# loicland/superpoint_graph

Measured on AMD Instinct MI355X. Metric: superpoints/sec (embed+ECC fwd+bwd), S3DIS-shaped SPG, higher is better.
Workload: dtype f32; 1 GPU; gru_10_0,f_13 fwd+bwd+Adam; 1 scene/GPU x 1000 sp x 128 pts x 14 f, 5000 edges x 13 f; hipgraph=False, step_call=spg_train_step (one library call: forward + backward), parallelism=single GPU, batchnorm=per-rank statistics, precision=f32

## Files before the change

### include/spg_hip.h

```cpp
#ifndef SPG_HIP_H
#define SPG_HIP_H
#include <stddef.h>
#include <stdint.h>

#ifdef __cplusplus
extern "C" {
#endif

#define SPG_MAX_LAYERS 8
#define SPG_VERSION 200

const char* spg_last_error(void);
int spg_version(void);

size_t spg_graph_workspace_bytes(int N, int n_src, int E);
int spg_graph_build(const int64_t* idxn, const int64_t* degs, int N, int n_src, int E, void* graph_ws, void* stream);
int spg_graph_export(const void* graph_ws, int N, int n_src, int E, int32_t* rowptr, int32_t* src, int32_t* dst,
                     int32_t* rev_rowptr, int32_t* rev_eid, int32_t* hdr, void* stream);

int spg_ecc_aggregate_fwd(int dtype, const void* x, const void* w, const int64_t* idxe, const void* graph_ws, int N,
                          int E, int cin, int cout, int w_is_matrix, void* out, void* stream);
int spg_ecc_aggregate_bwd(int dtype, const void* x, const void* w, const int64_t* idxe, const void* graph_ws, int N,
                          int E, int n_x_rows, int n_w_rows, int cin, int cout, int w_is_matrix, const void* grad_out,
                          void* grad_x, void* grad_w, void* stream);
// ... 47 lines not shown
                             const float* ext_transform, const void* const* params, float* emb, void* workspace, int training,
                             int bn_update_times, void* stream);
int spg_pointnet_backward_ext(const spg_pointnet_cfg* cfg, int B, const float* clouds, const float* clouds_global,
                              const float* ext_transform, const void* const* params, const float* grad_emb, void* const* grads,
                              float* grad_transform, float* grad_global, void* workspace, void* bwd_workspace, void* stream);

#define SPG_MAX_PARTS 64
typedef struct spg_eccrnn_cfg {
  int nc, nrepeats, matrix, layernorm, ingate, cat_all;
  int n_fnet;
  int fnet_widths[SPG_MAX_LAYERS + 1];
  int bnidx, llbias;
  float bn_eps, bn_momentum;
  int cell;
  int n_parts;
  int part_ptr[SPG_MAX_PARTS + 1];
} spg_eccrnn_cfg;

size_t spg_eccrnn_workspace_bytes(const spg_eccrnn_cfg* cfg, int N, int E, int training);
int spg_eccrnn_forward(const spg_eccrnn_cfg* cfg, int N, int E, const void* graph_ws, const float* h0,
                       const float* edgefeats, const void* const* params, float* out, void* workspace, int training,
                       int bn_update_times, void* stream);
long spg_eccrnn_debug_offset(const spg_eccrnn_cfg* cfg, int N, int E, int training, int layer, int what);
size_t spg_eccrnn_bwd_workspace_bytes(const spg_eccrnn_cfg* cfg, int N, int E);
int spg_eccrnn_backward(const spg_eccrnn_cfg* cfg, int N, int E, const void* graph_ws, const float* edgefeats,
                        const void* const* params, const float* grad_out, float* grad_h0, void* const* grads,
                        void* workspace, void* bwd_workspace, void* stream);

#define SPG_LOADER_MAX_FEATS 16
int spg_load_superpoints(const float* points, int ncols, const int64_t* offsets, int n_superpoints, const int32_t* slot,
                         const int32_t* sample_idx, int npts, int xyznormalize, const int32_t* colmap, int nfeat,
                         const double* M, const float* noise, float* clouds, float* diam, void* stream);

size_t spg_set_batch_workspace_bytes(int N, int E);
int spg_set_batch(const int64_t* edges, int N, int E, int64_t* idxn, int64_t* degs, int64_t* perm, void* workspace,
                  int32_t* error_flag, void* stream);
int spg_gather_rows(const float* src, long ld_src, const int64_t* perm, long rows, int cols, float* dst, long ld_dst,
                    void* stream);

enum { SPG_EF_COPY = 0, SPG_EF_DIFF = 1, SPG_EF_LOGDIFF = 2, SPG_EF_RATIO = 3, SPG_EF_CONST = 4 };
#define SPG_EF_MAX_COLS 32
typedef struct {
  const void* data;
  long ld;
  int column, kind, is_f64, pad_;
} spg_edge_feature_spec;
typedef struct {
  int ncols, pad_;
  spg_edge_feature_spec col[SPG_EF_MAX_COLS];
} spg_edge_feature_specs;
int spg_edge_features(const spg_edge_feature_specs* specs, const int64_t* edges, long E, const double* mean,
                      const double* scale, float* out, void* stream);

size_t spg_batch_graph_scratch_bytes(int N, int E, int F);
int spg_batch_graph_build(const int64_t* edges_host, const float* feats_host, int N, int E, int F, int64_t* idxn, int64_t* degs,
                          float* feats_sorted, void* graph_ws, void* scratch, int32_t* error_flag, void* stream);
int spg_batch_graph_build_dev(const int64_t* edges_dev, const float* feats_dev, int N, int E, int F, int64_t* idxn, int64_t* degs,
                              float* feats_sorted, void* graph_ws, void* scratch, int32_t* error_flag, void* stream);
int spg_upload_packed(const void* const* host, const size_t* bytes, const size_t* offsets, int n, void* device, size_t total, void* stream);

int spg_upload(const void* host, size_t bytes, void* device, void* stream);

size_t spg_spg_workspace_bytes(int which, long n);
int spg_spg_tet_edges(const int32_t* tets, long T, const int32_t* comp, uint64_t* keys, long capacity, uint64_t* count, void* stream);
int spg_spg_unique_edges(const uint64_t* keys, long n, const float* xyz, const int32_t* comp, long n_com, float d_max,
                         uint64_t* edge_keys, uint64_t* cc_keys, uint64_t* count, void* workspace, size_t workspace_bytes, void* stream);
int spg_spg_group_edges(const uint64_t* cc_keys, const uint64_t* edge_keys, long n, uint64_t* cc_sorted, uint64_t* edges_sorted,
                        uint64_t* seg_cc, int64_t* seg_off, int64_t* n_seg, void* workspace, size_t workspace_bytes, void* stream);
int spg_spg_superpoints(const float* xyz, long n, const int32_t* comp, int n_com, const int32_t* labels, const uint32_t* label_rows,
                        int n_labels, float* centroids, float* length, float* surface, float* volume, uint64_t* point_count,
                        uint32_t* sp_labels, void* workspace, size_t workspace_bytes, void* stream);
int spg_spg_superedges(const uint64_t* edges_sorted, const uint64_t* seg_cc, const int64_t* seg_off, long n_sedg, long n_com,
                       const float* xyz, const float* centroids, const float* length, const float* surface, const float* volume,
                       const uint64_t* point_count, uint32_t* source, uint32_t* target, float* delta_mean, float* delta_std,
                       float* delta_norm, float* delta_centroid, float* length_ratio, float* surface_ratio, float* volume_ratio,
                       float* point_count_ratio, void* stream);
int spg_compute_geof(const float* xyz, const uint32_t* target, long n, int k_nn, float* geof, void* stream);

size_t spg_prune_workspace_bytes(long n);
int spg_prune_voxels(const float* xyz, long n, float voxel_size, int64_t* n_voxels, int32_t* error_flag, void* workspace,
                     size_t workspace_bytes, void* stream);
int spg_prune_reduce(const float* xyz, const uint8_t* rgb, const uint8_t* labels, const uint32_t* objects, long n, long n_voxels,
                     int n_labels, int n_objects, float* out_xyz, uint8_t* out_rgb, uint32_t* out_labels, uint32_t* out_objects,
                     int32_t* error_flag, void* workspace, size_t workspace_bytes, void* stream);

size_t spg_knn_workspace_bytes(long n_ref, long n_query, int k);
int spg_knn_build(const float* ref_xyz, long n_ref, float cell_size, int32_t* error_flag, void* workspace, size_t workspace_bytes,
                  void* stream);
int spg_knn_query(const float* query_xyz, long n_query, long n_ref, int k, int self_query, int32_t* idx_out, float* dist_out,
                  int32_t* error_flag, void* workspace, size_t workspace_bytes, void* stream);
long spg_knn_query_chunk(long n_ref, long n_query, size_t workspace_bytes);

size_t spg_edgegraph_workspace_bytes(long n, long E);
int spg_edgegraph_build(const int64_t* src, const int64_t* tgt, long E, long n, int32_t* rowptr, uint32_t* inc, int32_t* ends,
                        int32_t* error_flag, void* workspace, size_t workspace_bytes, void* stream);
size_t spg_edge_forward_workspace_bytes(long E);
int spg_edge_forward(int mode, const float* emb, long n, int d, const int32_t* ends, long E, int dist_type, int intra, int inter,
                     const uint8_t* is_transition, const float* weights, float* diff, float* dx, float* dl, double* loss_out,
                     void* workspace, size_t workspace_bytes, void* stream);
int spg_edge_loss_backward(const float* dl, const uint8_t* is_transition, const float* up, long E, float* grad_diff, void* stream);
int spg_edge_backward(const float* emb, long n, int d, const int32_t* rowptr, const uint32_t* inc, const int32_t* ends, long E,
                      int dist_type, const float* dl, const uint8_t* is_transition, const float* up, const float* grad_diff,
                      const float* dx, float* grad_emb, void* stream);
size_t spg_cc_workspace_bytes(long n);
int spg_connected_components(const int32_t* ends, const uint8_t* active, long E, long n, int32_t* in_component,
                             int32_t* component_size, int32_t* n_components, void* workspace, size_t workspace_bytes, void* stream);
size_t spg_xpart_workspace_bytes(long n, long E);
int spg_xpart_weights(const int32_t* ends, long E, long n, const int32_t* pred_in_component, const uint8_t* is_transition,
                      double factor, float* weights, int32_t* in_component, int32_t* component_size, int32_t* n_components,
                      void* workspace, size_t workspace_bytes, void* stream);

int spg_loader_random(const int64_t* counts, const int64_t* ids, const int32_t* slot, int n_superpoints, int npts, int nfeat,
                      uint64_t seed, uint32_t step, int augment, float scale, int rot, float mirror_prob, int jitter,
                      int32_t* sample_idx, double* M, float* noise, void* stream);

int spg_cross_entropy_fwd(const float* logits, const int64_t* target, const float* weight, int N, int C, int64_t ignore_index,
                          int reduction_mean, float* loss, float* lse, float* wsum, void* stream);
int spg_cross_entropy_bwd(const float* logits, const int64_t* target, const float* weight, const float* lse, const float* wsum,
                          const float* grad_loss, int N, int C, int64_t ignore_index, int reduction_mean, float* grad_logits,
                          void* stream);

int spg_eval_accumulate(const float* logits, int n_samples, long sample_stride, int N, int C, const int64_t* label_mode,
                        const int64_t* label_vec, int64_t* pred, int64_t* confusion, int64_t* counters, void* stream);

typedef int (*spg_allreduce_fn)(void* ctx, double* buf, long n, void* stream);
int spg_set_bn_allreduce(spg_allreduce_fn fn, void* ctx, double* buf, long buf_doubles);
typedef int (*spg_slot_allreduce_fn)(void* ctx, unsigned long long* words, long nwords, void* stream);
int spg_set_slot_allreduce(spg_slot_allreduce_fn fn, void* ctx, int world);

int spg_rccl_unique_id(void* out_128_bytes);
int spg_rccl_init(const void* unique_id_128_bytes, int world_size, int rank);
int spg_rccl_world_size(void);
int spg_rccl_allreduce_sum_f32(float* buf, long n, void* stream);
int spg_rccl_sync_bn(double* buf, long buf_doubles);
int spg_rccl_sync_slots(int on);
int spg_rccl_allreduce_sum_f64(double* buf, long n, void* stream);
int spg_rccl_destroy(void);

int spg_adam_clamp_step(float* param, float* grad, float* exp_avg, float* exp_avg_sq, long n, float lr, float beta1,
                        float beta2, float eps, float weight_decay, float grad_clip, int step, void* stream);
int spg_adam_clamp_step_scaled(float* param, float* grad, float* exp_avg, float* exp_avg_sq, long n, float lr, float beta1,
                               float beta2, float eps, float weight_decay, float grad_clip, int step, const float* grad_div,
                               void* stream);
int spg_adam_clamp_step_guarded(float* param, float* grad, float* exp_avg, float* exp_avg_sq, long n, float lr, float beta1,
                                float beta2, float eps, float weight_decay, float grad_clip, int step, const float* grad_div,
                                const float* guard_all, void* stream);
int spg_ecc_persistent_flag(float* dst, void* stream);

void spg_prof_enable(int on);
int spg_prof_read(double* ms, long* launches, double* flops, int reset);
int spg_prof_tag(int kind, int it, int jt, int x, int y, int full);
int spg_prof_read_shapes(int* keys, double* vals, int max);
int spg_tune(int key, int value);
typedef struct spg_step_args {
  const spg_pointnet_cfg* ptn_cfg;
  int B, bn_update_times;
  const float* clouds;
  const float* clouds_global;
  const void* const* ptn_params;
  void* const* ptn_grads;
  void* ptn_ws; void* ptn_bwd_ws;
  float* emb;
  float* grad_emb;
  int N, nf;
  const int64_t* slot_of_row;
  const int64_t* idx_valid;
  float* desc;
  float* grad_desc;
  const spg_eccrnn_cfg* ecc_cfg;
  int E;
  const void* graph_ws;
  const float* edgefeats;
  const void* const* ecc_params;
  void* const* ecc_grads;
  void* ecc_ws; void* ecc_bwd_ws;
  float* ecc_out;
  float* grad_ecc_out;
  int nout, n_classes;
  const float* cls_W; const float* cls_b;
  float* cls_dW; float* cls_db;
  float* cls_work;
  float* logits;
  float* grad_logits;
  const int64_t* target;
  const float* class_weight;
  int64_t ignore_index;
  int reduction_mean;
  float* loss_buf;
  int ptn_slots_clean;
} spg_step_args;
int spg_train_step(const spg_step_args* args, void* stream);
int spg_infer_step(const spg_step_args* args, void* stream);
int spg_cross_entropy_fwd_bwd(const float* logits, const int64_t* target, const float* weight, int N, int C, int64_t ignore_index,
                              int reduction_mean, float* loss, float* lse, float* wsum, float* grad_logits, void* stream);

int spg_ecc_persistent_errors(void);
int spg_ecc_persistent_errors_clear(void);
int spg_ecc_persistent_status(int* errors, int* withheld, int clear);
int spg_prof_read_tag(int tag, double* ms, long* launches, double* flops);

int spg_group_trace(void* buf, int max_launches);
int spg_group_trace_read(int* out, int max);

#ifdef __cplusplus
}
#endif
#endif
```

### superpoint_graph_amd/_lib.py

```python
from __future__ import annotations

import ctypes
import os
import subprocess

import torch

_HERE = os.path.dirname(os.path.abspath(__file__))
CSRC = os.path.join(_HERE, 'csrc')
LIB_PATH = os.environ.get('SPG_HIP_LIB') or os.path.join(CSRC, 'libspg_hip.so')

SPG_MAX_LAYERS = 8
SPG_MAX_PARTS = 64
c_void_pp = ctypes.POINTER(ctypes.c_void_p)


class PointNetCfg(ctypes.Structure):
    _fields_ = [('nfeat', ctypes.c_int), ('nfeat_stn', ctypes.c_int), ('nfeat_global', ctypes.c_int), ('npts', ctypes.c_int),
                ('n_stn_conv', ctypes.c_int), ('n_stn_fc', ctypes.c_int), ('n_conv', ctypes.c_int), ('n_fc', ctypes.c_int),
                ('stn_conv', ctypes.c_int * SPG_MAX_LAYERS), ('stn_fc', ctypes.c_int * SPG_MAX_LAYERS),
                ('conv', ctypes.c_int * SPG_MAX_LAYERS), ('fc', ctypes.c_int * SPG_MAX_LAYERS),
                ('last_ac', ctypes.c_int), ('bn_eps', ctypes.c_float), ('bn_momentum', ctypes.c_float)]


class EccRnnCfg(ctypes.Structure):
    _fields_ = [('nc', ctypes.c_int), ('nrepeats', ctypes.c_int), ('matrix', ctypes.c_int), ('layernorm', ctypes.c_int),
                ('ingate', ctypes.c_int), ('cat_all', ctypes.c_int), ('n_fnet', ctypes.c_int),
                ('fnet_widths', ctypes.c_int * (SPG_MAX_LAYERS + 1)), ('bnidx', ctypes.c_int), ('llbias', ctypes.c_int),
                ('bn_eps', ctypes.c_float), ('bn_momentum', ctypes.c_float), ('cell', ctypes.c_int),
                ('n_parts', ctypes.c_int), ('part_ptr', ctypes.c_int * (SPG_MAX_PARTS + 1))]


_i, _l, _p, _sz = ctypes.c_int, ctypes.c_long, ctypes.c_void_p, ctypes.c_size_t

SPG_EF_MAX_COLS = 32


class EdgeFeatureSpec(ctypes.Structure):
    _fields_ = [('data', ctypes.c_void_p), ('ld', ctypes.c_long), ('column', ctypes.c_int), ('kind', ctypes.c_int),
                ('is_f64', ctypes.c_int), ('pad_', ctypes.c_int)]


class StepArgs(ctypes.Structure):
    _fields_ = [('ptn_cfg', ctypes.POINTER(PointNetCfg)), ('B', ctypes.c_int), ('bn_update_times', ctypes.c_int),
                ('clouds', ctypes.c_void_p), ('clouds_global', ctypes.c_void_p), ('ptn_params', c_void_pp), ('ptn_grads', c_void_pp),
                ('ptn_ws', ctypes.c_void_p), ('ptn_bwd_ws', ctypes.c_void_p), ('emb', ctypes.c_void_p), ('grad_emb', ctypes.c_void_p),
                ('N', ctypes.c_int), ('nf', ctypes.c_int), ('slot_of_row', ctypes.c_void_p), ('idx_valid', ctypes.c_void_p),
                ('desc', ctypes.c_void_p), ('grad_desc', ctypes.c_void_p),
                ('ecc_cfg', ctypes.POINTER(EccRnnCfg)), ('E', ctypes.c_int), ('graph_ws', ctypes.c_void_p), ('edgefeats', ctypes.c_void_p),
                ('ecc_params', c_void_pp), ('ecc_grads', c_void_pp), ('ecc_ws', ctypes.c_void_p), ('ecc_bwd_ws', ctypes.c_void_p),
                ('ecc_out', ctypes.c_void_p), ('grad_ecc_out', ctypes.c_void_p),
                ('nout', ctypes.c_int), ('n_classes', ctypes.c_int), ('cls_W', ctypes.c_void_p), ('cls_b', ctypes.c_void_p),
                ('cls_dW', ctypes.c_void_p), ('cls_db', ctypes.c_void_p), ('cls_work', ctypes.c_void_p), ('logits', ctypes.c_void_p),
                ('grad_logits', ctypes.c_void_p),
                ('target', ctypes.c_void_p), ('class_weight', ctypes.c_void_p), ('ignore_index', ctypes.c_int64),
                ('reduction_mean', ctypes.c_int), ('loss_buf', ctypes.c_void_p), ('ptn_slots_clean', ctypes.c_int)]


class EdgeFeatureSpecs(ctypes.Structure):
    _fields_ = [('ncols', ctypes.c_int), ('pad_', ctypes.c_int), ('col', EdgeFeatureSpec * SPG_EF_MAX_COLS)]


SIGNATURES = {
    'spg_last_error': (ctypes.c_char_p, []),
    'spg_version': (_i, []),
    'spg_graph_workspace_bytes': (_sz, [_i, _i, _i]),
    'spg_graph_build': (_i, [_p, _p, _i, _i, _i, _p, _p]),
    'spg_graph_export': (_i, [_p, _i, _i, _i, _p, _p, _p, _p, _p, _p, _p]),
    'spg_ecc_aggregate_fwd': (_i, [_i, _p, _p, _p, _p, _i, _i, _i, _i, _i, _p, _p]),
    'spg_ecc_aggregate_bwd': (_i, [_i, _p, _p, _p, _p, _i, _i, _i, _i, _i, _i, _i, _p, _p, _p, _p]),
    'spg_gru_scratch_floats': (_sz, [_i]),
    'spg_gru_cell_fwd': (_i, [_p, _p, _i, c_void_pp, _i, _i, _p, _p, _p]),
    'spg_gru_cell_bwd': (_i, [_p, _p, _p, _i, c_void_pp, _i, _i, _p, _p, c_void_pp, _p, _p]),
    'spg_lstm_scratch_floats': (_sz, [_i]),
    'spg_lstm_cell_fwd': (_i, [_p, _p, _p, _i, c_void_pp, _i, _i, _p, _p, _p, _p]),
    'spg_lstm_cell_bwd': (_i, [_p, _p, _p, _p, _p, _i, c_void_pp, _i, _i, _p, _p, _p, c_void_pp, _p, _p]),
    'spg_linear_fwd': (_i, [_p, _l, _i, _i, _p, _p, _i, _p, _p, _i, _p, _l, _p]),
    'spg_linear_dgrad': (_i, [_p, _l, _i, _i, _p, _i, _p, _l, _p]),
    'spg_colsum': (_i, [_p, _l, _l, _i, _p, _p, _p]),
    'spg_linear_wgrad_work_floats': (_sz, [_i, _i, _i]),
    'spg_linear_wgrad': (_i, [_p, _l, _p, _l, _i, _i, _i, _p, _p, _i, _p, _p, _p]),
    'spg_linear_wgrad_bias_work_floats': (ctypes.c_size_t, [_i, _i, _i]),
    'spg_linear_wgrad_bias': (_i, [_p, _l, _p, _l, _i, _i, _i, _p, _p, _i, _p, _p, _p, _p]),
    'spg_linear_backward': (_i, [_p, _l, _p, _l, _p, _i, _i, _i, _p, _l, _p, _p, _p, _p]),
    'spg_pointnet_num_layers': (_i, [ctypes.POINTER(PointNetCfg)]),
    'spg_pointnet_workspace_bytes': (_sz, [ctypes.POINTER(PointNetCfg), _i, _i]),
    'spg_pointnet_forward': (_i, [ctypes.POINTER(PointNetCfg), _i, _p, _p, c_void_pp, _p, _p, _i, _i, _p]),
    'spg_pointnet_forward_ext': (_i, [ctypes.POINTER(PointNetCfg), _i, _p, _p, _p, c_void_pp, _p, _p, _i, _i, _p]),
    'spg_pointnet_backward_ext': (_i, [ctypes.POINTER(PointNetCfg), _i, _p, _p, _p, c_void_pp, _p, c_void_pp, _p, _p, _p, _p, _p]),
    'spg_pointnet_debug_offset': (_l, [ctypes.POINTER(PointNetCfg), _i, _i, _i, _i]),
    'spg_pointnet_bwd_workspace_bytes': (_sz, [ctypes.POINTER(PointNetCfg), _i]),
    'spg_pointnet_backward': (_i, [ctypes.POINTER(PointNetCfg), _i, _p, _p, c_void_pp, _p, c_void_pp, _p, _p, _p]),
    'spg_eccrnn_workspace_bytes': (_sz, [ctypes.POINTER(EccRnnCfg), _i, _i, _i]),
    'spg_eccrnn_forward': (_i, [ctypes.POINTER(EccRnnCfg), _i, _i, _p, _p, _p, c_void_pp, _p, _p, _i, _i, _p]),
    'spg_eccrnn_bwd_workspace_bytes': (_sz, [ctypes.POINTER(EccRnnCfg), _i, _i]),
    'spg_eccrnn_debug_offset': (_l, [ctypes.POINTER(EccRnnCfg), _i, _i, _i, _i, _i]),
    'spg_ecc_persistent_errors': (_i, []),
    'spg_ecc_persistent_errors_clear': (_i, []),
    'spg_ecc_persistent_status': (_i, [ctypes.POINTER(ctypes.c_int), ctypes.POINTER(ctypes.c_int), _i]),
    'spg_eccrnn_backward': (_i, [ctypes.POINTER(EccRnnCfg), _i, _i, _p, _p, c_void_pp, _p, _p, c_void_pp, _p, _p, _p]),
    'spg_adam_clamp_step': (_i, [_p, _p, _p, _p, _l, ctypes.c_float, ctypes.c_float, ctypes.c_float, ctypes.c_float,
                                 ctypes.c_float, ctypes.c_float, _i, _p]),
    'spg_adam_clamp_step_scaled': (_i, [_p, _p, _p, _p, _l, ctypes.c_float, ctypes.c_float, ctypes.c_float, ctypes.c_float,
                                        ctypes.c_float, ctypes.c_float, _i, _p, _p]),
    'spg_adam_clamp_step_guarded': (_i, [_p, _p, _p, _p, _l, ctypes.c_float, ctypes.c_float, ctypes.c_float, ctypes.c_float,
                                        ctypes.c_float, ctypes.c_float, _i, _p, _p, _p]),
    'spg_ecc_persistent_flag': (_i, [_p, _p]),
    'spg_load_superpoints': (_i, [_p, _i, _p, _i, _p, _p, _i, _i, _p, _i, _p, _p, _p, _p, _p]),
    'spg_set_batch_workspace_bytes': (_sz, [_i, _i]),
    'spg_set_batch': (_i, [_p, _i, _i, _p, _p, _p, _p, _p, _p]),
    'spg_gather_rows': (_i, [_p, _l, _p, _l, _i, _p, _l, _p]),
    'spg_upload': (_i, [_p, _sz, _p, _p]),
    'spg_batch_graph_scratch_bytes': (_sz, [_i, _i, _i]),
    'spg_batch_graph_build': (_i, [_p, _p, _i, _i, _i, _p, _p, _p, _p, _p, _p, _p]),
    'spg_batch_graph_build_dev': (_i, [_p, _p, _i, _i, _i, _p, _p, _p, _p, _p, _p, _p]),
    'spg_upload_packed': (_i, [_p, _p, _p, _i, _p, _sz, _p]),
    'spg_spg_workspace_bytes': (_sz, [_i, _l]),
    'spg_spg_tet_edges': (_i, [_p, _l, _p, _p, _l, _p, _p]),
    'spg_spg_unique_edges': (_i, [_p, _l, _p, _p, _l, ctypes.c_float, _p, _p, _p, _p, _sz, _p]),
    'spg_spg_group_edges': (_i, [_p, _p, _l, _p, _p, _p, _p, _p, _p, _sz, _p]),
    'spg_spg_superpoints': (_i, [_p, _l, _p, _i, _p, _p, _i, _p, _p, _p, _p, _p, _p, _p, _sz, _p]),
    'spg_spg_superedges': (_i, [_p, _p, _p, _l, _l] + [_p] * 16 + [_p]),
    'spg_compute_geof': (_i, [_p, _p, _l, _i, _p, _p]),
    'spg_prune_workspace_bytes': (_sz, [_l]),
    'spg_prune_voxels': (_i, [_p, _l, ctypes.c_float, _p, _p, _p, _sz, _p]),
    'spg_prune_reduce': (_i, [_p, _p, _p, _p, _l, _l, _i, _i, _p, _p, _p, _p, _p, _p, _sz, _p]),
    'spg_knn_workspace_bytes': (_sz, [_l, _l, _i]),
    'spg_knn_build': (_i, [_p, _l, ctypes.c_float, _p, _p, _sz, _p]),
    'spg_knn_query': (_i, [_p, _l, _l, _i, _i, _p, _p, _p, _p, _sz, _p]),
    'spg_knn_query_chunk': (_l, [_l, _l, _sz]),
    'spg_edgegraph_workspace_bytes': (_sz, [_l, _l]),
    'spg_edgegraph_build': (_i, [_p, _p, _l, _l, _p, _p, _p, _p, _p, _sz, _p]),
    'spg_edge_forward_workspace_bytes': (_sz, [_l]),
    'spg_edge_forward': (_i, [_i, _p, _l, _i, _p, _l, _i, _i, _i, _p, _p, _p, _p, _p, _p, _p, _sz, _p]),
    'spg_edge_loss_backward': (_i, [_p, _p, _p, _l, _p, _p]),
    'spg_edge_backward': (_i, [_p, _l, _i, _p, _p, _p, _l, _i, _p, _p, _p, _p, _p, _p, _p]),
    'spg_cc_workspace_bytes': (_sz, [_l]),
    'spg_connected_components': (_i, [_p, _p, _l, _l, _p, _p, _p, _p, _sz, _p]),
    'spg_xpart_workspace_bytes': (_sz, [_l, _l]),
    'spg_xpart_weights': (_i, [_p, _l, _l, _p, _p, ctypes.c_double, _p, _p, _p, _p, _p, _sz, _p]),
    'spg_edge_features': (_i, [ctypes.POINTER(EdgeFeatureSpecs), _p, _l, _p, _p, _p, _p]),
    'spg_loader_random': (_i, [_p, _p, _p, _i, _i, _i, ctypes.c_uint64, ctypes.c_uint32, _i, ctypes.c_float, _i, ctypes.c_float, _i, _p, _p, _p, _p]),
    'spg_cross_entropy_fwd': (_i, [_p, _p, _p, _i, _i, ctypes.c_int64, _i, _p, _p, _p, _p]),
    'spg_cross_entropy_bwd': (_i, [_p, _p, _p, _p, _p, _p, _i, _i, ctypes.c_int64, _i, _p, _p]),
    'spg_cross_entropy_fwd_bwd': (_i, [_p, _p, _p, _i, _i, ctypes.c_int64, _i, _p, _p, _p, _p, _p]),
    'spg_train_step': (_i, [ctypes.POINTER(StepArgs), _p]),
    'spg_infer_step': (_i, [ctypes.POINTER(StepArgs), _p]),
    'spg_eval_accumulate': (_i, [_p, _i, _l, _i, _i, _p, _p, _p, _p, _p, _p]),
    'spg_set_bn_allreduce': (_i, [_p, _p, _p, _l]),
    'spg_rccl_unique_id': (_i, [_p]),
    'spg_rccl_init': (_i, [_p, _i, _i]),
    'spg_rccl_world_size': (_i, []),
    'spg_rccl_allreduce_sum_f32': (_i, [_p, _l, _p]),
    'spg_rccl_sync_bn': (_i, [_p, _l]),
    'spg_rccl_sync_slots': (_i, [_i]),
    'spg_group_trace': (_i, [_p, _i]),
    'spg_group_trace_read': (_i, [_p, _i]),
    'spg_rccl_allreduce_sum_f64': (_i, [_p, _l, _p]),
    'spg_set_slot_allreduce': (_i, [_p, _p, _i]),
    'spg_rccl_destroy': (_i, []),
    'spg_prof_enable': (None, [_i]),
    'spg_prof_tag': (_i, [_i, _i, _i, _i, _i, _i]),
    'spg_prof_read_tag': (_i, [_i, ctypes.POINTER(ctypes.c_double), ctypes.POINTER(ctypes.c_long), ctypes.POINTER(ctypes.c_double)]),
    'spg_prof_read_shapes': (_i, [ctypes.POINTER(_i), ctypes.POINTER(ctypes.c_double), _i]),
    'spg_tune': (_i, [_i, _i]),
    'spg_prof_read': (_i, [ctypes.POINTER(ctypes.c_double), ctypes.POINTER(ctypes.c_long), ctypes.POINTER(ctypes.c_double), _i]),
}

_lib = None


def build(verbose: bool = False) -> str:
    out = subprocess.run(['make', '-C', CSRC, '-j8'], capture_output=True, text=True)
    if out.returncode != 0:
        raise RuntimeError('building libspg_hip.so failed:\n' + out.stdout[-4000:] + out.stderr[-4000:])
    if verbose:
        print(out.stdout[-2000:])
    return LIB_PATH


def lib():
    global _lib
    if _lib is None:
        if not os.path.exists(LIB_PATH):
            raise RuntimeError(f'{LIB_PATH} not found: the HIP extension is not built '
                               f'(run `python -c "import __graft_entry__ as g; g.build()"` or `make -C {CSRC}`). '
                               'There is no CPU fallback for the product path.')
        L = ctypes.CDLL(LIB_PATH)
        for name, (res, args) in SIGNATURES.items():
            fn = getattr(L, name)
            fn.restype = res
            fn.argtypes = args
        _lib = L
    return _lib


def check(rc: int, what: str = ''):
    if rc != 0:
        msg = lib().spg_last_error()
        raise RuntimeError(f'libspg_hip {what} failed (rc={rc}): {msg.decode() if msg else ""}')
```

### superpoint_graph_amd/csrc/spg_common.h

```cpp
#pragma once
#include <float.h>
#include <hip/hip_runtime.h>
#include <stdint.h>
#include <stdio.h>
#include <string.h>

typedef float f32x16 __attribute__((ext_vector_type(16)));
typedef float f32x4 __attribute__((ext_vector_type(4)));

#define SPG_KC 32
#define SPG_MAX_DEVICES 16
#define SPG_THREADS 256

extern "C" const char* spg_last_error(void);
void spg_set_error(const char* fmt, ...);
enum { SPG_TUNE_NO_PERSIST = 0, SPG_TUNE_DBG = 3, SPG_TUNE_FIN_SLICE_MIN = 4, SPG_TUNE_NO_STAT_ACCUM = 5, SPG_TUNE_NO_HEAD_SERVICE = 6, SPG_TUNE_PRECISION = 7,
       SPG_TUNE_NO_PERSIST_ECC = 8, SPG_TUNE_NO_BN_FOLD = 10, SPG_TUNE_NO_GROUP = 11, SPG_TUNE_NO_BWD_PAIR = 14, SPG_TUNE_NO_ECC_HEAD = 15, SPG_TUNE_NO_NARROW_PAIR = 17, SPG_TUNE_NO_FIRST_CONV_BWD = 18, SPG_TUNE_PX_SPIN_LIMIT = 20, SPG_TUNE_NO_ADAM_GUARD = 21, SPG_TUNE_NO_PAIR_SPLIT = 22, SPG_TUNE_COUNT = 23 };
int spg_tune_get(int key);

#define SPG_CHECK_ARG(cond, msg)                                          \
  do {                                                                    \
    if (!(cond)) {                                                        \
      spg_set_error("%s:%d: bad argument: %s", __FILE__, __LINE__, msg);  \
      return -1;                                                          \
    }                                                                     \
  } while (0)

#define SPG_LAUNCH_CHECK()                                                                  \
  do {                                                                                      \
    hipError_t e__ = hipGetLastError();                                                     \
    if (e__ != hipSuccess) {                                                                \
      spg_set_error("%s:%d: launch failed: %s", __FILE__, __LINE__, hipGetErrorString(e__)); \
      return (int)e__;                                                                      \
    }                                                                                       \
  } while (0)

#define SPG_TRY(expr)           \
  do {                          \
    int rc__ = (expr);          \
    if (rc__ != 0) return rc__; \
  } while (0)

static inline int spg_cdiv(long a, long b) { return (int)((a + b - 1) / b); }

enum {
  SPG_PRO_IDENT = 0,
  SPG_PRO_AFFINE = 1,
  SPG_PRO_CLOUD = 2,
  SPG_PRO_BNBWD = 3,
  SPG_PRO_POOLBWD = 4
};

struct SpgOperand {
  const float* X;
  const float* X2;
  long ld;
  const float* c0;
  const float* c1;
  const float* c2;
  const float* c3;
  const int* aidx;
  const float* stnT;
  int mode;
  int relu;
  int n_affine;
  int Ctot;
  int P;
  int ldg;
};

__device__ __forceinline__ float spg_bnbwd_value(float a, float x, float b, float y, float c, float d) {
  return fmaf(a, x - b, -__fmul_rn(y - c, d));
}

typedef float spg_f32x2 __attribute__((ext_vector_type(2)));
typedef float spg_f32x4 __attribute__((ext_vector_type(4)));
__device__ __forceinline__ spg_f32x4 spg_fma4(spg_f32x4 a, spg_f32x4 b, spg_f32x4 c) { return __builtin_elementwise_fma(a, b, c); }
__device__ __forceinline__ spg_f32x2 spg_fma2(spg_f32x2 a, spg_f32x2 b, spg_f32x2 c) { return __builtin_elementwise_fma(a, b, c); }
__device__ __forceinline__ spg_f32x4 spg_bnbwd_value4(spg_f32x4 a, spg_f32x4 x, spg_f32x4 b, spg_f32x4 y, spg_f32x4 c, spg_f32x4 d) {
#pragma clang fp contract(off)
  const spg_f32x4 t = (y - c) * d;
  const spg_f32x4 u = x - b;
  return __builtin_elementwise_fma(a, u, -t);
}

__device__ __forceinline__ float spg_fetch(const SpgOperand& d, long m, int c) {
  switch (d.mode) {
    case SPG_PRO_IDENT:
      return d.X[m * d.ld + c];
    case SPG_PRO_AFFINE: {
      float v = d.X[m * d.ld + c];
      if (c < d.n_affine) {
        if (d.c0) v = fmaf(v, d.c0[c], d.c1[c]);
        if (d.relu) v = fmaxf(v, 0.f);
      }
      return v;
    }
    case SPG_PRO_CLOUD: {
      long g = m / d.P;
      int p = (int)(m - g * d.P);
      const float* base = d.X + (g * d.Ctot) * (long)d.P + p;
      if (d.stnT != nullptr && c < 2) {
        const float* T = d.stnT + g * 4;
        float x = base[0], y = base[d.P];
        return c == 0 ? fmaf(x, T[0] + 1.f, y * T[2]) : fmaf(x, T[1], y * (T[3] + 1.f));
      }
      return base[(long)c * d.P];
    }
    case SPG_PRO_BNBWD: {
      float dz = d.X[m * d.ld + c];
      float y = d.X2[m * d.ld + c];
      return spg_bnbwd_value(d.c0[c], dz, d.c1[c], y, d.c2[c], d.c3[c]);
    }
    default: {
      long g = m / d.P;
      int p = (int)(m - g * d.P);
      float dz = (d.aidx[g * d.ldg + c] == p) ? d.X[g * d.ldg + c] : 0.f;
      float y = d.X2[m * d.ld + c];
      return spg_bnbwd_value(d.c0[c], dz, d.c1[c], y, d.c2[c], d.c3[c]);
    }
  }
}

struct SpgQuad {
  f32x4 a, b, c, d;
  int nvalid;
  int naff;
  int relu;
  int has;
};

__host__ __device__ inline bool spg_operand_vec_ok(const SpgOperand& d) {
  if (d.mode == SPG_PRO_CLOUD) return false;
  if ((d.ld & 3) != 0 || (((uintptr_t)d.X) & 15) != 0) return false;
  if ((d.mode == SPG_PRO_BNBWD || d.mode == SPG_PRO_POOLBWD) && (((uintptr_t)d.X2) & 15) != 0) return false;
  if (d.mode == SPG_PRO_POOLBWD && ((d.ldg & 3) != 0 || (((uintptr_t)d.aidx) & 15) != 0)) return false;
  if (d.mode == SPG_PRO_AFFINE &&
      ((d.n_affine & 3) != 0 || (d.c0 != nullptr && ((((uintptr_t)d.c0) | ((uintptr_t)d.c1)) & 15) != 0))) return false;
  if ((d.mode == SPG_PRO_BNBWD || d.mode == SPG_PRO_POOLBWD) &&
      ((((uintptr_t)d.c0) | ((uintptr_t)d.c1) | ((uintptr_t)d.c2) | ((uintptr_t)d.c3)) & 15) != 0) return false;
  return true;
}

template <int MODE>
__device__ __forceinline__ SpgQuad spg_quad_consts(const SpgOperand& d, int c, int nch) {
  SpgQuad q;
  q.nvalid = nch - c < 0 ? 0 : (nch - c > 4 ? 4 : nch - c);
  q.naff = 0; q.relu = 0; q.has = 0;
  if (MODE == SPG_PRO_AFFINE) {
    const int lim = d.n_affine < nch ? d.n_affine : nch;
    q.naff = c + 4 <= lim ? 4 : 0;
    q.relu = d.relu;
    q.has = d.c0 != nullptr;
    const float* p0 = q.has ? d.c0 : d.X;
    const float* p1 = q.has ? d.c1 : d.X;
    const int cb = (q.has && q.naff) ? c : 0;
    q.a = *reinterpret_cast<const f32x4*>(p0 + cb);
    q.b = *reinterpret_cast<const f32x4*>(p1 + cb);
  } else if (MODE == SPG_PRO_BNBWD || MODE == SPG_PRO_POOLBWD) {
    const int cb = c < nch ? c : 0;
    q.a = *reinterpret_cast<const f32x4*>(d.c0 + cb);
    q.b = *reinterpret_cast<const f32x4*>(d.c1 + cb);
    q.c = *reinterpret_cast<const f32x4*>(d.c2 + cb);
    q.d = *reinterpret_cast<const f32x4*>(d.c3 + cb);
  } else if (MODE == SPG_PRO_CLOUD) {
    q.naff = (d.stnT != nullptr && c == 0) ? 1 : 0;
  }
  return q;
}

// ... 949 lines not shown
```

### superpoint_graph_amd/csrc/spg_gemm.h

```cpp
#pragma once
#include "spg_common.h"

enum { SPG_EPI_FWD = 0, SPG_EPI_BWD = 1 };

#ifndef SPG_FOLD_SLOTS
#define SPG_FOLD_SLOTS 4
#endif
#define SPG_FOLD_MAX_CONTRIBUTIONS ((long)SPG_FOLD_SLOTS << 17)
inline size_t spg_fold_slot_words(int C) { return (size_t)SPG_FOLD_SLOTS * 4 * C + 8; }
struct SpgBnFold {
  const unsigned long long* slots;
  int C, update_times;
  float momentum, eps;
  double count;
  const float *gamma, *beta;
  float *rm, *rv;
  float *mean, *rstd, *s, *t;
};
struct SpgBnFoldBwd {
  const unsigned long long* slots;
  int C;
  double count;
  const float *s, *mean, *rstd;
  float* consts;
  float *dgamma, *dbeta;
  double grad_mul;
};
bool spg_slot_sync_active();
int spg_slot_sync_world();
int spg_slot_sync_after(unsigned long long* slots, size_t words, hipStream_t stream, bool deferred);
#define SPG_FC_ROWS 32

struct SpgGemmParams {
  SpgOperand a;
  const float* W;
  long ldw;
  int w_red;
  const float* bias;
  int M, N, K;
  int rows_per_tile;
  int epi;
  float* Y;
  long ldy;
  float* stat;
  float* stat_cnt;
  unsigned long long* stat_slots;
  long stat_rows;
  SpgBnFold fold;
  SpgBnFoldBwd fold_bwd;
  float* pool_out;
  int* pool_idx;
  const float* pool_sign;
  const float* pool_extra;
  long pool_ld;
  int pool_nextra;
  const float* Yp;
  long ldyp;
  const float* ms;
  const float* mt;
  int vec_store;
  int mask_relu;
  int n_mask;
  const float* mmean;
  const float* mrstd;
  int remap, ncol, ntile, rstride;
  int stat_accum;
  int dbg;
  const void* Wb;
  long ldwb, wb_part_bytes;
};

struct SpgWgradParams {
  SpgOperand a;
  SpgOperand b;
  int M, N, K;
  int rows_per_split;
  float* partial;
  float* colsum;
  SpgBnFoldBwd fold;
  int allow_lowp;
};

struct SpgSplitJob { const float* W; long ldw; int N, K; void* fwd; void* bwd; };
#define SPG_SPLIT_MAX_JOBS 40
struct SpgSplitBatch { SpgSplitJob jobs[SPG_SPLIT_MAX_JOBS]; int njobs = 0; };
inline long spg_split_ld(int k) { return (k + 7) & ~7; }
inline size_t spg_split_bytes(int rows, int cols) { return (size_t)2 * rows * spg_split_ld(cols) * 2; }
int spg_launch_split_weights(const SpgSplitBatch& b, hipStream_t stream);
int spg_gemm_precision();

struct SpgGroupScope {
  explicit SpgGroupScope(hipStream_t stream);
  ~SpgGroupScope();
  int flush();
  bool active() const { return owner_; }
  SpgGroupScope(const SpgGroupScope&) = delete;
  SpgGroupScope& operator=(const SpgGroupScope&) = delete;
 private:
  bool owner_;
};
struct SpgGroupBypass {
  explicit SpgGroupBypass(bool on = true);
  ~SpgGroupBypass();
 private:
  bool on_;
};
int spg_group_zero(float* p, size_t n, hipStream_t stream);

#include <functional>
typedef std::function<int(hipStream_t)> SpgStage;
void spg_riders_push(SpgStage stage);
int spg_riders_pending();
int spg_riders_drain(hipStream_t stream);
void spg_riders_clear();

struct SpgProfSpan {
  SpgProfSpan(hipStream_t stream, double flops, int tag, int N, int K);
  ~SpgProfSpan();
  SpgProfSpan(const SpgProfSpan&) = delete;
  SpgProfSpan& operator=(const SpgProfSpan&) = delete;
 private:
  void* impl_;
};

int spg_gemm_ntiles(const SpgGemmParams& p);
inline bool spg_gemm_bwd_stats_want_partials(const SpgGemmParams& g) { return g.w_red && g.N > 64 && g.rows_per_tile > SPG_FC_ROWS && !spg_slot_sync_active(); }
int spg_gemm_row_waves(int rows_per_tile, int N);
int spg_launch_gemm(const SpgGemmParams& p, hipStream_t stream, int* stat_parts = nullptr);

size_t spg_wgrad_workspace_floats(long M, int N, int K);
size_t spg_wgrad_colsum_floats(long M, int N, int K);
int spg_launch_wgrad(SpgWgradParams p, float* dW, float* work, hipStream_t stream);

#define SPG_MAX_REDUCE_JOBS 40
struct SpgReduceJob {
  const float* partial;
  float* out;
  int nsplit, n;
};
struct SpgReduceQueue {
  SpgReduceJob jobs[SPG_MAX_REDUCE_JOBS];
  int njobs = 0;
  float* arena = nullptr;
  size_t arena_floats = 0, used = 0;
};
int spg_queue_wgrad(SpgReduceQueue& q, SpgWgradParams p, float* dW, hipStream_t stream, float* db = nullptr);
bool spg_bwdpair_supported(const SpgGemmParams& g, const SpgOperand& b);
int spg_queue_bwdpair(SpgReduceQueue& q, SpgGemmParams g, const SpgOperand& b, float* dW, hipStream_t stream);
int spg_queue_partials(SpgReduceQueue& q, int nsplit, int n, float* out, float** partial, hipStream_t stream);
int spg_queue_colsum(SpgReduceQueue& q, const float* X, long ld, long M, int N, float* out, hipStream_t stream);
int spg_flush_reduce(SpgReduceQueue& q, hipStream_t stream);
void spg_reduce_defer(const SpgReduceJob& job);
void spg_reduce_deferred_clear();
int spg_flush_deferred_reduce(hipStream_t stream);
int spg_reduce_ride(SpgReduceQueue& q, hipStream_t stream, size_t max_bytes = (size_t)36 << 20);

size_t spg_bn_finalize_scratch_doubles(int N);
int spg_launch_bn_finalize(const float* stat, const float* stat_cnt, int nparts, long M, int N, const float* gamma,
                           const float* beta, float* running_mean, float* running_var, float momentum, float eps,
                           int update_times, float* mean, float* rstd, float* s, float* t, double* scratch,
                           hipStream_t stream);
bool spg_sync_bn_active();
struct SpgBnEvalJob { int N; const float *gamma, *beta, *rm, *rv; float *s, *t; };
#define SPG_BN_EVAL_MAX_JOBS 40
struct SpgBnEvalBatch { SpgBnEvalJob jobs[SPG_BN_EVAL_MAX_JOBS]; int njobs = 0; };
int spg_launch_bn_eval_batch(const SpgBnEvalBatch& b, float eps, hipStream_t stream);
int spg_launch_bn_eval(int N, const float* gamma, const float* beta, const float* running_mean,
                       const float* running_var, float eps, float* s, float* t, hipStream_t stream);
int spg_launch_bn_bwd_finalize(const float* stat, int ntile, int ldstat, long count, int N, const float* s,
                               const float* mean, const float* rstd, float* consts, float* dgamma, float* dbeta,
                               double* scratch, hipStream_t stream);
int spg_launch_pool_select(const float* pmax, const float* pmin, const int* imax, const int* imin, const float* s,
                           int G, int N, int rows_per_tile, const float* extra, int nextra, float* out, long ldo, int* aidx,
                           hipStream_t stream);
size_t spg_colsum_workspace_floats(int N);
int spg_launch_colsum(const float* X, long ld, long M, int N, float* out, float* work, hipStream_t stream);
int spg_launch_pad_rows(const float* src, long lds, float* dst, long ldd, long rows, int cols, hipStream_t stream);
int spg_launch_stn_dT(const float* clouds, int Ctot, int P, int G, const float* dxy, long ldd, float* dT,
                      hipStream_t stream);


#define SPG_CONVSTACK_MAX_LAYERS 8
struct SpgConvStackParams {
  const float* clouds;
  const float* stnT;
  int B, P, Ctot, nlayers;
  int cin[SPG_CONVSTACK_MAX_LAYERS], cout[SPG_CONVSTACK_MAX_LAYERS];
  const float *W[SPG_CONVSTACK_MAX_LAYERS], *bias[SPG_CONVSTACK_MAX_LAYERS];
  f32x4* Wp[SPG_CONVSTACK_MAX_LAYERS];
  const float *s[SPG_CONVSTACK_MAX_LAYERS], *t[SPG_CONVSTACK_MAX_LAYERS];
  float *pmax, *pmin;
};
int spg_launch_pool_select_parts(const float* pmax, const float* pmin, const int* imax, const int* imin, const float* s,
                                 int G, int N, int nparts, const float* extra, int nextra, float* out, long ldo, int* aidx,
                                 hipStream_t stream);
size_t spg_conv_stack_packed_floats(int cin, int cout);
bool spg_conv_stack_eval_supported(const SpgConvStackParams& p);
int spg_launch_conv_stack_eval(const SpgConvStackParams& p, hipStream_t stream);
```

### superpoint_graph_amd/csrc/spg_gemm.hip

```cpp
#pragma clang fp contract(off)
#include "../../include/spg_hip.h"
#include "spg_gemm.h"
#include <type_traits>
#include <float.h>
#include <limits.h>
#include <stdarg.h>

static thread_local char g_err[512] = "";
extern "C" const char* spg_last_error(void) { return g_err; }
void spg_set_error(const char* fmt, ...) {
  va_list ap;
  va_start(ap, fmt);
  vsnprintf(g_err, sizeof(g_err), fmt, ap);
  va_end(ap);
}

#include <mutex>
#include <vector>
#ifdef SPG_ATTRIBUTION
#define SPG_DBG(p) ((p).dbg)
#else
#define SPG_DBG(p) 0
#endif
namespace {
struct ProfRec { hipEvent_t a, b; double flops; int tag; int M, N, K; };
bool g_prof_on = false;
std::vector<ProfRec> g_prof;
std::mutex g_prof_mutex;
struct ProfScope {
  hipStream_t st; bool on; ProfRec r;
  ProfScope(hipStream_t s, double flops, int tag = 0, bool enable = true) : st(s), on(g_prof_on && enable) {
    if (on) { (void)hipEventCreate(&r.a); (void)hipEventCreate(&r.b); r.flops = flops; r.tag = tag; r.M = r.N = r.K = 0; (void)hipEventRecord(r.a, st); }
  }
  ~ProfScope() { if (on) { (void)hipEventRecord(r.b, st); std::lock_guard<std::mutex> lock(g_prof_mutex); g_prof.push_back(r); } }
};
}
extern "C" void spg_prof_enable(int on) { g_prof_on = on != 0; }
SpgProfSpan::SpgProfSpan(hipStream_t stream, double flops, int tag, int N, int K) : impl_(nullptr) {
  if (!g_prof_on) return;
  ProfScope* ps = new ProfScope(stream, flops, tag);
  ps->r.N = N; ps->r.K = K;
  impl_ = ps;
}
SpgProfSpan::~SpgProfSpan() { delete static_cast<ProfScope*>(impl_); }

static int g_tune[SPG_TUNE_COUNT] = {0};
static int spg_num_cus() {
  static int n = 0;
  if (n == 0) {
    int dev = 0, v = 0;
    if (hipGetDevice(&dev) == hipSuccess && hipDeviceGetAttribute(&v, hipDeviceAttributeMultiprocessorCount, dev) == hipSuccess && v > 0) n = v;
    else n = 256;
  }
  return n;
}
int spg_tune_get(int key) { return (key >= 0 && key < SPG_TUNE_COUNT) ? g_tune[key] : 0; }
extern "C" int spg_tune(int key, int value) {
  if (key < 0 || key >= SPG_TUNE_COUNT) return -1;
  if ((key == 9 || key == 12 || key == 13 || key == 16 || key == 19) && value != 0) return -1;
#ifndef SPG_ATTRIBUTION
  if ((key == SPG_TUNE_DBG || key == SPG_TUNE_NO_STAT_ACCUM) && value != 0) return -1;
#endif
  const int old = g_tune[key];
  g_tune[key] = value;
  return old;
}

namespace { thread_local int g_riding = 0; }
struct SpgRidingScope { SpgRidingScope() { ++g_riding; } ~SpgRidingScope() { --g_riding; } };
#define SPG_OWNER_WEIGHT 100000

extern "C" int spg_prof_read_shapes(int* keys, double* vals, int max) {
  std::lock_guard<std::mutex> lock(g_prof_mutex);
  int n = 0;
  for (ProfRec& r : g_prof) {
    (void)hipEventSynchronize(r.b);
    float dt = 0.f;
    (void)hipEventElapsedTime(&dt, r.a, r.b);
    int j = 0;
    for (; j < n; ++j)
      if (keys[4 * j] == r.tag && keys[4 * j + 1] == r.N && keys[4 * j + 2] == r.K) break;
    if (j == n) {
      if (n == max) continue;
      keys[4 * n] = r.tag; keys[4 * n + 1] = r.N; keys[4 * n + 2] = r.K; keys[4 * n + 3] = 0;
      vals[2 * n] = 0.0; vals[2 * n + 1] = 0.0;
      ++n;
    }
    keys[4 * j + 3] += 1; vals[2 * j] += dt; vals[2 * j + 1] += r.flops;
  }
  return n;
}
#define SPG_PROF_TAG(kind, IT, JT, X, Y, FULL) ((kind) * 1000000 + ((IT) / 32) * 100000 + ((JT) / 32) * 10000 + ((X) + 1) * 100 + ((Y) + 1) * 10 + (FULL))
extern "C" int spg_prof_tag(int kind, int it, int jt, int x, int y, int full) { return SPG_PROF_TAG(kind, it, jt, x, y, full ? 1 : 0); }
extern "C" int spg_prof_read_tag(int tag, double* ms, long* launches, double* flops) {
  std::lock_guard<std::mutex> lock(g_prof_mutex);
  double t = 0.0, f = 0.0;
  long n = 0;
  for (ProfRec& r : g_prof) {
    if (r.tag != tag) continue;
    (void)hipEventSynchronize(r.b);
    float dt = 0.f;
    (void)hipEventElapsedTime(&dt, r.a, r.b);
    t += dt; f += r.flops; ++n;
  }
  if (ms) *ms = t;
  if (launches) *launches = n;
  if (flops) *flops = f;
  return 0;
}
extern "C" int spg_prof_read(double* ms, long* launches, double* flops, int reset) {
  std::lock_guard<std::mutex> lock(g_prof_mutex);
  double t = 0.0, f = 0.0;
  for (ProfRec& r : g_prof) {
    (void)hipEventSynchronize(r.b);
    float dt = 0.f;
    (void)hipEventElapsedTime(&dt, r.a, r.b);
    t += dt; f += r.flops;
  }
  if (ms) *ms = t;
  if (launches) *launches = (long)g_prof.size();
  if (flops) *flops = f;
  if (reset) {
    for (ProfRec& r : g_prof) { (void)hipEventDestroy(r.a); (void)hipEventDestroy(r.b); }
    g_prof.clear();
  }
  return 0;
}

#include "spg_ecc.h"
enum { SPG_JOB_GEMM = 1, SPG_JOB_WGRAD = 2, SPG_JOB_COLSUM = 3, SPG_JOB_EDGE_WGRAD = 4, SPG_JOB_PAD_ROWS = 5, SPG_JOB_ZERO = 6, SPG_JOB_REDUCE = 7 };
struct SpgSmallJob {
  const float* src;
  float* dst;
  long a, b, c;
  int i;
};
struct SpgJobHdr { int kind, variant, gx, gy, gz, offset, weight, reserved; };
#define SPG_GROUP_MAX_JOBS 16
#define SPG_GROUP_ARENA_BYTES 3440
#define SPG_GROUP_MAX_WGRAD_ROWS 65536
struct SpgMultiArgs {
  int njobs, pad;
  unsigned long long* trace;
  int first_block[SPG_GROUP_MAX_JOBS];
  SpgJobHdr hdr[SPG_GROUP_MAX_JOBS];
  alignas(16) unsigned char arena[SPG_GROUP_ARENA_BYTES];
};
static_assert(sizeof(SpgMultiArgs) <= 4096, "kernel arguments of a grouped launch must fit 4 KiB");
static_assert(sizeof(SpgGemmParams) % 8 == 0 && sizeof(SpgWgradParams) % 8 == 0, "parameter structs are packed back to back");
constexpr int spg_gemm_variant(bool wred, int amode, bool full) {
  const int m = amode == -1 ? (full ? -1 : 4)
              : amode == SPG_PRO_IDENT ? (full ? 1 : 0)
              : ((!wred && amode == SPG_PRO_AFFINE) || (wred && amode == SPG_PRO_BNBWD)) ? (full ? 3 : 2) : -1;
  return m < 0 ? -1 : (wred ? 5 : 0) + m;
}
constexpr bool spg_gemm_variant_light(int v) { return v != 8; }
#define SPG_WGRAD_VARIANTS(X)                                                                                    \
  X(0, 128, 128, 2, 2, 3, 1, false, false, false)   X(1, 128, 128, 2, 2, 3, 1, true, false, false)               \
  X(2, 64, 64, 2, 2, 0, 1, false, true, true)       X(3, 64, 64, 2, 2, 0, 1, true, true, true)                   \
  X(4, 128, 64, 2, 2, 0, 1, false, false, false)    X(5, 128, 64, 2, 2, 0, 1, true, false, false)                \
  X(6, 128, 128, 2, 2, -1, -1, false, true, false)                                                               \
  X(7, 128, 32, 4, 1, 0, 0, false, false, true)     X(8, 128, 32, 4, 1, 0, 0, true, false, true)                 \
  X(9, 128, 32, 4, 1, -1, -1, false, true, false)                                                                \
  X(10, 128, 32, 4, 1, 0, 0, false, true, false)    X(11, 128, 32, 4, 1, 0, 0, true, true, true)                 \
  X(12, 128, 32, 4, 1, 0, 1, false, true, false)    X(13, 128, 32, 4, 1, 0, 1, true, true, false)                \
  X(14, 64, 64, 2, 2, 0, 1, false, false, true)     X(15, 64, 64, 2, 2, 0, 1, true, false, true)                 \
  X(16, 128, 128, 2, 2, 0, 1, false, true, false)   X(17, 128, 128, 2, 2, 0, 1, true, true, false)               \
  X(18, 128, 64, 2, 2, 3, 1, false, false, false)   X(19, 128, 64, 2, 2, 3, 1, true, false, false)
constexpr int spg_wgrad_variant(int it, int jt, int amode, int bmode, bool full, bool colsum) {
#define SPG_X(id, IT_, JT_, WI_, WJ_, AM_, BM_, FU_, CS_, LI_) \
  if (it == IT_ && jt == JT_ && amode == AM_ && bmode == BM_ && full == FU_ && colsum == CS_) return id;
  SPG_WGRAD_VARIANTS(SPG_X)
#undef SPG_X
  return -1;
}
constexpr bool spg_wgrad_variant_light(int v) {
#define SPG_X(id, IT_, JT_, WI_, WJ_, AM_, BM_, FU_, CS_, LI_) if (v == id) return LI_;
  SPG_WGRAD_VARIANTS(SPG_X)
#undef SPG_X
  return false;
}
static bool spg_group_accepts(hipStream_t stream);
static bool spg_group_add(int kind, int variant, const void* params, size_t bytes, dim3 grid, size_t lds, double flops, hipStream_t stream, int weight,
                          std::function<int()> direct = nullptr);

__device__ __forceinline__ int spg_opaque_zero() { int z = 0; asm volatile("" : "+v"(z)); return z; }
template <typename T> using spg_kernarg_ptr = __attribute__((address_space(4))) const T*;
template <int BYTES>
__device__ __forceinline__ void spg_touch_params(const spg_kernarg_ptr<unsigned> b) {
  unsigned acc = 0;
#pragma unroll
  for (int o = 0; o < BYTES; o += 64) acc |= b[o / 4];
  asm volatile("" :: "s"(acc));
}
#define SPG_EPI_PIECE_ROWS 16
#define SPG_EPI_WAVE_FLOATS(RW, CW) (SPG_EPI_PIECE_ROWS * ((CW) + 8))

template <int RW, int CW, int TI, int TJ>
__device__ __forceinline__ void spg_store_tile_vec_impl(const f32x16 (&acc)[TI][TJ], float* __restrict__ st,
                                                        float* __restrict__ ybase, unsigned ldy, int lane) {
  constexpr int LD = CW + 8, LPR = CW / 4, RPI = 64 / LPR;
  static_assert(SPG_EPI_PIECE_ROWS % RPI == 0, "a piece is a whole number of store instructions");
  const int r = lane & 31, h = lane >> 5;
  const int lr = lane / LPR, lc = 4 * (lane % LPR);
  const unsigned o0 = (unsigned)lr * ldy + (unsigned)lc;
#pragma unroll
  for (int i = 0; i < TI; ++i)
#pragma unroll
    for (int half = 0; half < 2; ++half) {
#pragma unroll
      for (int j = 0; j < TJ; ++j)
#pragma unroll
        for (int u = 0; u < 8; ++u) st[((u & 3) + 8 * (u >> 2) + 4 * h) * LD + 32 * j + r] = acc[i][j][8 * half + u];
#pragma unroll
      for (int it = 0; it < SPG_EPI_PIECE_ROWS / RPI; ++it) {
// ... 1321 lines not shown
    const long n = (long)p.N * p.K;
    hipLaunchKernelGGL(spg_reduce_partials_kernel, dim3(spg_cdiv(n, 64)), dim3(1024), 0, stream, work, ns, n, dW);
    SPG_LAUNCH_CHECK();
  }
  return 0;
}

struct SpgReduceBatch {
  SpgReduceJob jobs[SPG_MAX_REDUCE_JOBS];
  int first_block[SPG_MAX_REDUCE_JOBS + 1];
  int njobs;
};

#define SPG_REDUCE_ELEMS 256
__global__ __launch_bounds__(1024) void spg_reduce_batch_kernel(const SpgReduceBatch b) {
  __shared__ f32x4 red[16][64];
  int j = 0;
  while (j + 1 < b.njobs && (int)blockIdx.x >= b.first_block[j + 1]) ++j;
  const SpgReduceJob job = b.jobs[j];
  const int tx = threadIdx.x & 63, ty = threadIdx.x >> 6;
  const long i = ((long)(blockIdx.x - b.first_block[j]) * 64 + tx) * 4;
  f32x4 s = {0.f, 0.f, 0.f, 0.f};
  const bool vec = (job.n & 3) == 0 && ((((uintptr_t)job.out) | ((uintptr_t)job.partial)) & 15) == 0;
  if (vec) {
    if (i < job.n) {
      int k = ty;
      for (; k + 48 < job.nsplit; k += 64) {
        const f32x4 v0 = *reinterpret_cast<const f32x4*>(job.partial + (long)k * job.n + i);
        const f32x4 v1 = *reinterpret_cast<const f32x4*>(job.partial + (long)(k + 16) * job.n + i);
        const f32x4 v2 = *reinterpret_cast<const f32x4*>(job.partial + (long)(k + 32) * job.n + i);
        const f32x4 v3 = *reinterpret_cast<const f32x4*>(job.partial + (long)(k + 48) * job.n + i);
        s += v0; s += v1; s += v2; s += v3;
      }
      for (; k < job.nsplit; k += 16) s += *reinterpret_cast<const f32x4*>(job.partial + (long)k * job.n + i);
    }
  } else {
    for (int e = 0; e < 4; ++e)
      if (i + e < job.n)
        for (int k = ty; k < job.nsplit; k += 16) s[e] += job.partial[(long)k * job.n + i + e];
  }
  red[ty][tx] = s;
  __syncthreads();
  if (ty == 0 && i < job.n) {
    f32x4 t = {0.f, 0.f, 0.f, 0.f};
#pragma unroll
    for (int k = 0; k < 16; ++k) t += red[k][tx];
    if (vec) {
      *reinterpret_cast<f32x4*>(job.out + i) = t;
    } else {
      for (int e = 0; e < 4; ++e)
        if (i + e < job.n) job.out[i + e] = t[e];
    }
  }
}

namespace { thread_local std::vector<SpgReduceJob> g_deferred_reduce; }
void spg_reduce_defer(const SpgReduceJob& job) { g_deferred_reduce.push_back(job); }
void spg_reduce_deferred_clear() { g_deferred_reduce.clear(); }

static int launch_reduce_jobs(const SpgReduceJob* jobs, int n, hipStream_t stream) {
  for (int base = 0; base < n; base += SPG_MAX_REDUCE_JOBS) {
    const int m = n - base < SPG_MAX_REDUCE_JOBS ? n - base : SPG_MAX_REDUCE_JOBS;
    SpgReduceBatch b;
    int blocks = 0;
    for (int j = 0; j < m; ++j) {
      b.jobs[j] = jobs[base + j];
      b.first_block[j] = blocks;
      blocks += spg_cdiv(jobs[base + j].n, SPG_REDUCE_ELEMS);
    }
    b.first_block[m] = blocks;
    b.njobs = m;
    hipLaunchKernelGGL(spg_reduce_batch_kernel, dim3(blocks), dim3(1024), 0, stream, b);
    SPG_LAUNCH_CHECK();
  }
  return 0;
}

int spg_flush_reduce(SpgReduceQueue& q, hipStream_t stream) {
  if (q.njobs == 0 && g_deferred_reduce.empty()) return 0;
  std::vector<SpgReduceJob> all(g_deferred_reduce);
  g_deferred_reduce.clear();
  all.insert(all.end(), q.jobs, q.jobs + q.njobs);
  q.njobs = 0;
  return launch_reduce_jobs(all.data(), (int)all.size(), stream);
}

int spg_reduce_ride(SpgReduceQueue& q, hipStream_t stream, size_t max_bytes) {
  if (!spg_group_accepts(stream)) return 0;
  SpgRidingScope riding;
  int kept = 0;
  size_t taken = 0;
  bool full = false;
  for (int j = 0; j < q.njobs; ++j) {
    const SpgReduceJob job = q.jobs[j];
    const size_t bytes = (size_t)job.nsplit * job.n * sizeof(float);
    if (!full && taken > 0 && taken + bytes > max_bytes) full = true;
    if (full || !spg_group_add(SPG_JOB_REDUCE, 0, &job, sizeof(job), dim3(spg_cdiv(job.n, 64)), 16 * 16 * sizeof(f32x4), 0.0, stream,
                               2 + job.nsplit / 32)) {
      q.jobs[kept++] = job;
      continue;
    }
    taken += bytes;
  }
  q.njobs = kept;
  return 0;
}

int spg_flush_deferred_reduce(hipStream_t stream) {
  SpgReduceQueue none;
  return spg_flush_reduce(none, stream);
}

static int queue_take(SpgReduceQueue& q, size_t floats, float** out, hipStream_t stream) {
  if (q.njobs == SPG_MAX_REDUCE_JOBS) SPG_TRY(spg_flush_reduce(q, stream));
  SPG_CHECK_ARG(q.arena != nullptr && q.used + floats <= q.arena_floats, "reduction arena too small");
  *out = q.arena + q.used;
  q.used += (floats + 63) & ~(size_t)63;
  return 0;
}

int spg_queue_partials(SpgReduceQueue& q, int nsplit, int n, float* out, float** partial, hipStream_t stream) {
  SPG_CHECK_ARG(nsplit >= 1 && n >= 1 && out != nullptr && partial != nullptr, "partials");
  if (q.njobs + 1 > SPG_MAX_REDUCE_JOBS) SPG_TRY(spg_flush_reduce(q, stream));
  SPG_TRY(queue_take(q, (size_t)nsplit * n, partial, stream));
  SpgReduceJob& j = q.jobs[q.njobs++];
  j.partial = *partial; j.out = out; j.nsplit = nsplit; j.n = n;
  return 0;
}

int spg_queue_wgrad(SpgReduceQueue& q, SpgWgradParams p, float* dW, hipStream_t stream, float* db) {
  SPG_CHECK_ARG(p.M > 0 && p.N > 0 && p.K > 0, "empty wgrad");
  int it, jt, ns, rps;
  wgrad_plan(p.M, p.N, p.K, &it, &jt, &ns, &rps);
  float* part = dW;
  if (q.njobs + 2 > SPG_MAX_REDUCE_JOBS) SPG_TRY(spg_flush_reduce(q, stream));
  if (ns > 1) SPG_TRY(queue_take(q, (size_t)ns * p.N * p.K, &part, stream));
  p.colsum = nullptr;
  if (db != nullptr) {
    p.colsum = db;
    if (ns > 1) SPG_TRY(queue_take(q, (size_t)ns * p.N, &p.colsum, stream));
  }
  SPG_TRY(spg_launch_wgrad_partials(p, part, stream));
  if (ns > 1) {
    SpgReduceJob& j = q.jobs[q.njobs++];
    j.partial = part; j.out = dW; j.nsplit = ns; j.n = p.N * p.K;
    if (db != nullptr) {
      SpgReduceJob& c = q.jobs[q.njobs++];
      c.partial = p.colsum; c.out = db; c.nsplit = ns; c.n = p.N;
    }
  }
  return 0;
}

template <int IT, int JT, int WI, int WJ>
__device__ __forceinline__ void spg_epilogue_bwd_vec_lds(const SpgGemmParams& p, f32x16 (&acc)[IT / WI / 32][JT / WJ / 32],
                                                         float* __restrict__ red, const float* __restrict__ ylds, int ldl, long m0,
                                                         SpgStatAcc<JT / WJ / 32>& sacc, const int pass) {
  constexpr int TI = IT / WI / 32, TJ = JT / WJ / 32, RW = IT / WI, CW = JT / WJ;
  constexpr int LD = CW + 8, LPR = CW / 4, RPI = 64 / LPR, NIT = SPG_EPI_PIECE_ROWS / RPI;
  const int tid = threadIdx.x + spg_opaque_zero(), lane = tid & 63, wave = (tid >> 6) & 3;
  const int r = lane & 31, h = lane >> 5;
  const int wi = wave / WJ, wj = wave % WJ;
  const int colw = wj * CW, roww = wi * RW;
  float* st = red + wave * SPG_EPI_WAVE_FLOATS(RW, CW);
  const int lr = lane / LPR, lc = 4 * (lane % LPR);
  const int col = colw + lc;
  const f32x4 sc = *reinterpret_cast<const f32x4*>(p.ms + col), sh = *reinterpret_cast<const f32x4*>(p.mt + col);
  const f32x4 mean = *reinterpret_cast<const f32x4*>(p.mmean + col), rstd = *reinterpret_cast<const f32x4*>(p.mrstd + col);
  const float* yl = ylds + (roww + lr) * ldl + col;
  float* yo = p.Y + (m0 + roww) * p.ldy + colw;
  const unsigned oo0 = (unsigned)lr * (unsigned)p.ldy + (unsigned)lc;
  f32x4 s1 = {0.f, 0.f, 0.f, 0.f}, s2 = s1;
  f32x4 prev[TI * 2 * NIT];
  if (pass == 2) {
#pragma unroll
    for (int i = 0; i < TI; ++i)
#pragma unroll
      for (int half = 0; half < 2; ++half)
#pragma unroll
        for (int u = 0; u < NIT; ++u)
          prev[(2 * i + half) * NIT + u] = *reinterpret_cast<const f32x4*>(yo + oo0 + (unsigned)(32 * i + 16 * half + RPI * u) * (unsigned)p.ldy);
  }
#pragma unroll
  for (int i = 0; i < TI; ++i)
#pragma unroll
    for (int half = 0; half < 2; ++half) {
      const int rb = 32 * i + 16 * half;
#pragma unroll
      for (int j = 0; j < TJ; ++j)
#pragma unroll
        for (int u = 0; u < 8; ++u) st[((u & 3) + 8 * (u >> 2) + 4 * h) * LD + 32 * j + r] = acc[i][j][8 * half + u];
#pragma unroll
      for (int u = 0; u < NIT; ++u) {
        f32x4 v = *reinterpret_cast<const f32x4*>(st + (lr + RPI * u) * LD + lc);
        if (pass == 2) v += prev[(2 * i + half) * NIT + u];
        if (pass != 1) {
          const f32x4 yv = *reinterpret_cast<const f32x4*>(yl + (rb + RPI * u) * ldl);
          const f32x4 act = spg_fma4(yv, sc, sh), xhat = (yv - mean) * rstd;
#pragma unroll
          for (int e = 0; e < 4; ++e)
            if (!(act[e] > 0.f)) v[e] = 0.f;
          s1 += v;
          s2 = spg_fma4(v, xhat, s2);
        }
        __builtin_nontemporal_store(v, reinterpret_cast<f32x4*>(yo + oo0 + (unsigned)(rb + RPI * u) * (unsigned)p.ldy));
      }
      __builtin_amdgcn_sched_barrier(0);
    }
  sacc.s1 += s1; sacc.s2 += s2;
}

struct SpgBwdPairParams {
  SpgGemmParams g;
  SpgOperand b;
  float* partial;
  int pass;
  int pad_;
};
#define SPG_PAIR_THREADS 1024
#ifdef SPG_ATTRIBUTION
__device__ unsigned long long spg_pair_role_t[3][3][4];
extern "C" int spg_pair_role_times(unsigned long long* out, int clear) {
  if (hipMemcpyFromSymbol(out, HIP_SYMBOL(spg_pair_role_t), sizeof(unsigned long long) * 36) != hipSuccess) return -1;
  if (clear) { unsigned long long z[36] = {0}; if (hipMemcpyToSymbol(HIP_SYMBOL(spg_pair_role_t), z, sizeof(z)) != hipSuccess) return -1; }
  return 0;
}
#define SPG_T0() unsigned long long t__ = __builtin_readcyclecounter(), tp__[4] = {0, 0, 0, t__ - tent__}
#define SPG_TENTRY() const unsigned long long tent__ = __builtin_readcyclecounter(); unsigned long long te__ = tent__, tq__[4] = {0, 0, 0, 0}
#define SPG_TQ(k) { const unsigned long long n__ = __builtin_readcyclecounter(); tq__[k] += n__ - te__; te__ = n__; }
#define SPG_TQEND() if (threadIdx.x == 0) { const int sh__ = (CO == 128) + (CI == 128); for (int k__ = 0; k__ < 4; ++k__) atomicAdd(&spg_pair_entry_t[sh__][k__], tq__[k__]); }
__device__ unsigned long long spg_pair_entry_t[3][4];
extern "C" int spg_pair_entry_times(unsigned long long* out, int clear) {
  if (hipMemcpyFromSymbol(out, HIP_SYMBOL(spg_pair_entry_t), sizeof(unsigned long long) * 12) != hipSuccess) return -1;
  if (clear) { unsigned long long z[12] = {0}; if (hipMemcpyToSymbol(HIP_SYMBOL(spg_pair_entry_t), z, sizeof(z)) != hipSuccess) return -1; }
  return 0;
}
#define SPG_TP(k) { const unsigned long long n__ = __builtin_readcyclecounter(); tp__[k] += n__ - t__; t__ = n__; }
#define SPG_TEND(role) if ((threadIdx.x & 255) == 0) { const int sh__ = (CO == 128) + (CI == 128); for (int k__ = 0; k__ < 4; ++k__) atomicAdd(&spg_pair_role_t[sh__][role][k__], tp__[k__]); }
#else
#define SPG_T0()
#define SPG_TENTRY()
#define SPG_TQ(k)
#define SPG_TQEND()
#define SPG_TP(k)
#define SPG_TEND(role)
#endif
template <int CO, int CI>
constexpr size_t spg_bwdpair_lds_bytes() {
  return 2 * ((size_t)(CO / 4) * (spg_bwdpair_rows(CI) + 1) * 16 + (size_t)spg_bwdpair_rows(CI) * (CI + 4) * 4) + (size_t)CO * (CI + 4) * 4 +
         (size_t)4 * SPG_EPI_WAVE_FLOATS(32, 32) * 4 + (size_t)(CO + CI / 2) * 16;
}

template <int CO, int CI, int AMODE>
__global__ __launch_bounds__(SPG_PAIR_THREADS) void spg_bwdpair_kernel(const SpgBwdPairParams p) {
  constexpr int IT = spg_bwdpair_rows(CI), SA = IT + 1, SX = CI + 4;
  constexpr int CQ = CO / 4, XQ = CI / 4;
  constexpr int NDZ = IT * CQ / 512, NX = IT * XQ / 512;
  constexpr int RDZ = 512 / CQ, RX = 512 / XQ;
  constexpr int WJ = CI / 32 > 4 ? 4 : CI / 32, WI = 4 / WJ;
  constexpr int TIW = CO / 32 / WI;
  constexpr int BUF4 = CQ * SA + IT * SX / 4;
  constexpr int TPG = 128 / IT;
  static_assert((CO == 64 || CO == 128) && (CI == 64 || CI == 128) && IT * WJ * 32 == 4096 * (WJ * 32 / CI), "supported shapes");
  static_assert(NDZ >= 1 && NX >= 1 && IT % RDZ == 0 && IT % RX == 0, "loader map");
  SPG_TENTRY();
  extern __shared__ f32x4 smem[];
  float* wl = reinterpret_cast<float*>(smem + 2 * BUF4);
  float* red = wl + CO * SX;
  f32x4* kst = reinterpret_cast<f32x4*>(red + 4 * SPG_EPI_WAVE_FLOATS(32, 32));
  const SpgGemmParams& g = p.g;
  const int tid = threadIdx.x, lane = tid & 63;
  const int wave = __builtin_amdgcn_readfirstlane(tid >> 6);
  const int r = lane & 31, h = lane >> 5;
  const int role = wave >> 2;
  const int wi = (wave & 3) / WJ, wj = (wave & 3) % WJ;
  const int ntile = g.ntile, stride = (int)gridDim.x;
  int tile = (int)blockIdx.x;

  auto prologue = [&](auto wload) __attribute__((always_inline)) {
    constexpr bool WLOAD = decltype(wload)::value;
    constexpr int NWQ = CO * XQ / 512;
    static_assert(CO * XQ % 512 == 0, "whole quads per thread");
    f32x4 wq[NWQ];
    if constexpr (WLOAD) {
#pragma unroll
      for (int k = 0; k < NWQ; ++k) {
        const int i = tid + k * 512, co = i / XQ, q = i % XQ;
        wq[k] = *reinterpret_cast<const f32x4*>(g.W + (long)co * g.ldw + 4 * q);
      }
    }
    if (g.stat_slots != nullptr && p.pass != 1 && blockIdx.x == 0 && tid == 0) spg_slots_count_add(g.stat_slots, g.n_mask, g.stat_rows != 0 ? g.stat_rows : (long)g.M);
    SPG_TQ(0);
    if (g.fold_bwd.slots != nullptr) spg_bn_fold_bwd(g.fold_bwd, blockIdx.x == 0);
    SPG_TQ(1);
    if (tid < CQ) {
      kst[0 * CQ + tid] = *reinterpret_cast<const f32x4*>(g.a.c0 + 4 * tid); kst[1 * CQ + tid] = *reinterpret_cast<const f32x4*>(g.a.c1 + 4 * tid);
      kst[2 * CQ + tid] = *reinterpret_cast<const f32x4*>(g.a.c2 + 4 * tid); kst[3 * CQ + tid] = *reinterpret_cast<const f32x4*>(g.a.c3 + 4 * tid);
    }
    if (tid < XQ) {
      kst[4 * CQ + tid] = *reinterpret_cast<const f32x4*>(p.b.c0 + 4 * tid); kst[4 * CQ + XQ + tid] = *reinterpret_cast<const f32x4*>(p.b.c1 + 4 * tid);
    }
    if constexpr (WLOAD) {
#pragma unroll
      for (int k = 0; k < NWQ; ++k) {
        const int i = tid + k * 512, co = i / XQ, q = i % XQ;
        *reinterpret_cast<f32x4*>(wl + co * SX + 4 * q) = wq[k];
      }
    }
    __syncthreads();
    SPG_TQ(2);
  };

  if (role >= 2) {
    const int lt = tid - 512;
    const int cq = lt % CQ, rdz = lt / CQ;
    const int xq = lt % XQ, rx = lt / XQ;
    const unsigned odz = ((unsigned)rdz * (unsigned)g.a.ld + 4u * (unsigned)cq) * 4u, sdz = (unsigned)RDZ * (unsigned)g.a.ld * 4u;
    const unsigned ox = ((unsigned)rx * (unsigned)p.b.ld + 4u * (unsigned)xq) * 4u, sx = (unsigned)RX * (unsigned)p.b.ld * 4u;
    struct Regs {
      f32x4 pg[AMODE == SPG_PRO_POOLBWD ? 1 : NDZ], py[NDZ], px[NX];
      int4 pai;
    };
    Regs R0, R1;
    auto load_tile = [&](Regs& R, int t) __attribute__((always_inline)) {
      const long m0 = (long)t * IT;
      if constexpr (AMODE == SPG_PRO_POOLBWD) {
        R.pg[0] = spg_ld16(g.a.X + (long)(t / TPG) * g.a.ldg, 16u * (unsigned)cq);
        R.pai = spg_ld16i(g.a.aidx + (long)(t / TPG) * g.a.ldg, 16u * (unsigned)cq);
      } else {
        const float* gb = g.a.X + m0 * g.a.ld;
#pragma unroll
        for (int i = 0; i < NDZ; ++i) R.pg[i] = spg_ld16(gb, odz + sdz * i);
      }
      const float* yb = g.a.X2 + m0 * g.a.ld;
#pragma unroll
      for (int i = 0; i < NDZ; ++i) R.py[i] = spg_ld16(yb, odz + sdz * i);
      const float* xb = p.b.X + m0 * p.b.ld;
#pragma unroll
      for (int i = 0; i < NX; ++i) R.px[i] = spg_ld16(xb, ox + sx * i);
    };
    auto store_tile = [&](const Regs& R, int t, int buf) __attribute__((always_inline)) {
      f32x4* dz4 = smem + buf * BUF4;
      float* xs = reinterpret_cast<float*>(dz4 + CQ * SA);
      const f32x4 ka = kst[0 * CQ + cq], kb = kst[1 * CQ + cq], kc = kst[2 * CQ + cq], kd = kst[3 * CQ + cq];
      const int prow = (t % TPG) * IT;
#pragma unroll
      for (int i = 0; i < NDZ; ++i) {
        const int row = rdz + RDZ * i;
        f32x4 gv;
        if constexpr (AMODE == SPG_PRO_POOLBWD) {
          gv[0] = R.pai.x == prow + row ? R.pg[0][0] : 0.f; gv[1] = R.pai.y == prow + row ? R.pg[0][1] : 0.f;
          gv[2] = R.pai.z == prow + row ? R.pg[0][2] : 0.f; gv[3] = R.pai.w == prow + row ? R.pg[0][3] : 0.f;
        } else {
          gv = R.pg[i];
        }
        dz4[cq * SA + row] = spg_bnbwd_value4(ka, gv, kb, R.py[i], kc, kd);
      }
#pragma unroll
      for (int i = 0; i < NX; ++i) *reinterpret_cast<f32x4*>(xs + (rx + RX * i) * SX + 4 * xq) = R.px[i];
    };
    constexpr bool LATE_R1 = 2 * sizeof(Regs) / 4 >= 64;
    load_tile(R0, tile);
    if (!LATE_R1 && tile + stride < ntile) load_tile(R1, tile + stride);
    prologue(std::false_type{});
    if (LATE_R1 && tile + stride < ntile) load_tile(R1, tile + stride);
    store_tile(R0, tile, 0);
    if (tile + 2 * stride < ntile) load_tile(R0, tile + 2 * stride);
    __syncthreads();
    SPG_T0();
    for (;;) {
      int nxt = tile + stride;
      bool has_next = nxt < ntile;
      if (has_next) {
        store_tile(R1, nxt, 1);
        SPG_TP(0);
        if (nxt + 2 * stride < ntile) load_tile(R1, nxt + 2 * stride);
        SPG_TP(1);
      }
      __syncthreads();
      SPG_TP(2);
      if (!has_next) break;
      tile = nxt;
      nxt = tile + stride;
      has_next = nxt < ntile;
      if (has_next) {
        store_tile(R0, nxt, 0);
        SPG_TP(0);
        if (nxt + 2 * stride < ntile) load_tile(R0, nxt + 2 * stride);
        SPG_TP(1);
      }
      __syncthreads();
      SPG_TP(2);
      if (!has_next) break;
      tile = nxt;
    }
    __syncthreads();
    SPG_TEND(2);
    return;
  }

  prologue(std::true_type{});
  if (role == 0) {
    f32x16 acc[1][1];
    SpgStatAcc<1> sacc;
    sacc.n = 0.f; sacc.a[0] = 0.f; sacc.b[0] = 0.f;
    sacc.s1 = f32x4{0.f, 0.f, 0.f, 0.f}; sacc.s2 = sacc.s1;
    __syncthreads();
    SPG_TQ(3); SPG_TQEND();
    int buf = 0;
    SPG_T0();
    for (;;) {
      const int nxt = tile + stride;
      const bool has_next = nxt < ntile;
      const f32x4* dz4 = smem + buf * BUF4;
#pragma unroll
      for (int q = 0; q < 16; ++q) acc[0][0][q] = 0.f;
      spg_mfma_tile_or<CO / 8, 2>(dz4, wl, SA, SX, wi * 32 + r, wj * 32 + r, h, acc[0][0]);
      SPG_TP(0);
      spg_epilogue_bwd_vec_lds<IT, CI, WI, WJ>(g, acc, red, reinterpret_cast<const float*>(dz4 + CQ * SA), SX, (long)tile * IT, sacc, p.pass);
      SPG_TP(1);
      __syncthreads();
      SPG_TP(2);
      if (!has_next) break;
      tile = nxt; buf ^= 1;
    }
    SPG_TEND(0);
    if (p.pass == 1) return;
    constexpr int CW = 32, LPR = CW / 4;
    float* xch = red;
    f32x4 s1 = sacc.s1, s2 = sacc.s2;
    const int cl = wj * CW + 4 * (lane % LPR);
#pragma unroll
    for (int off = LPR; off < 64; off <<= 1) {
#pragma unroll
      for (int e = 0; e < 4; ++e) { s1[e] += __shfl_xor(s1[e], off, 64); s2[e] += __shfl_xor(s2[e], off, 64); }
    }
    if (WI > 1 && wi != 0 && lane < LPR) {
      *reinterpret_cast<f32x4*>(xch + (wi * CI + cl) * 2) = s1;
      *reinterpret_cast<f32x4*>(xch + (wi * CI + cl) * 2 + 4) = s2;
    }
    __syncthreads();
    if (wi == 0 && lane < LPR) {
      if (WI > 1) {
        s1 += *reinterpret_cast<const f32x4*>(xch + (1 * CI + cl) * 2);
        s2 += *reinterpret_cast<const f32x4*>(xch + (1 * CI + cl) * 2 + 4);
      }
#pragma unroll
      for (int e = 0; e < 4; ++e) spg_slots_add(g.stat_slots, g.n_mask, cl + e, (double)s1[e], (double)s2[e]);
    }
    return;
  }

  f32x16 acc[TIW][1];
#pragma unroll
  for (int i = 0; i < TIW; ++i)
#pragma unroll
    for (int q = 0; q < 16; ++q) acc[i][0][q] = 0.f;
  const float xsc = reinterpret_cast<const float*>(kst + 4 * CQ)[wj * 32 + r], xsh = reinterpret_cast<const float*>(kst + 4 * CQ + XQ)[wj * 32 + r];
  __syncthreads();
  int buf = 0;
  SPG_T0();
  for (;;) {
    const int nxt = tile + stride;
    const bool has_next = nxt < ntile;
    const float* dzf = reinterpret_cast<const float*>(smem + buf * BUF4);
    const float* xs = dzf + CQ * SA * 4;
    spg_mfma_chunk_tr_aff<TIW, TIW, IT / 2>(dzf, xs, SA, SX, 0, wi * (32 * TIW) + r, wj * 32 + r, h, xsc, xsh, acc);
    SPG_TP(0);
    __syncthreads();
    SPG_TP(2);
    if (!has_next) break;
    tile = nxt; buf ^= 1;
  }
  SPG_TEND(1);
  __syncthreads();
  float* pb = p.partial + (long)blockIdx.x * CO * CI;
  const int kl = wj * 32 + r;
#pragma unroll
  for (int i = 0; i < TIW; ++i)
#pragma unroll
    for (int q = 0; q < 16; ++q) {
      const int nl = wi * (32 * TIW) + 32 * i + spg_acc_row(q, h);
      __builtin_nontemporal_store(acc[i][0][q], pb + nl * CI + kl);
    }
}

bool spg_bwdpair_supported(const SpgGemmParams& g, const SpgOperand& b) {
  if (g_tune[SPG_TUNE_NO_BWD_PAIR]) return false;
  const int CI = g.N, CO = g.K;
  if (!(g.w_red && g.epi == SPG_EPI_BWD && ((CI == 64 && (CO == 64 || CO == 128)) || (CI == 128 && (CO == 128 || (CO == 256 && !g_tune[SPG_TUNE_NO_PAIR_SPLIT] && g_tune[SPG_TUNE_PRECISION] == 0)))))) return false;
  const int IT = spg_bwdpair_rows(CI);
  if (g.M < IT || g.M % IT != 0) return false;
  const SpgOperand& a = g.a;
  if (a.mode != SPG_PRO_BNBWD && a.mode != SPG_PRO_POOLBWD) return false;
  if (!spg_operand_vec_ok(a) || a.ld < CO) return false;
  if (a.mode == SPG_PRO_POOLBWD && (a.P != 128 || a.ldg < CO)) return false;
  if (CO == 256 && g.fold_bwd.slots != nullptr && g.fold_bwd.C != CO) return false;
  if (b.mode != SPG_PRO_AFFINE || !b.relu || b.c0 == nullptr || b.n_affine != CI || !spg_operand_vec_ok(b) || b.ld < CI) return false;
  if ((g.ldw & 3) != 0 || (((uintptr_t)g.W) & 15) != 0 || g.ldw < CI) return false;
  if (g.Y == nullptr || g.Yp == nullptr || (g.ldy & 3) != 0 || (g.ldyp & 3) != 0 || ((((uintptr_t)g.Y) | ((uintptr_t)g.Yp)) & 15) != 0) return false;
  if (g.Yp != b.X || g.ldyp != b.ld) return false;
  if (g.stat_slots == nullptr || g.mmean == nullptr || g.mrstd == nullptr || g.ms == nullptr || g.mt == nullptr) return false;
  if (g.ms != b.c0 || g.mt != b.c1) return false;
  if (!g.mask_relu || g.n_mask != CI) return false;
  if ((((uintptr_t)g.ms) | ((uintptr_t)g.mt) | ((uintptr_t)g.mmean) | ((uintptr_t)g.mrstd)) & 15) return false;
  const long ntile = g.M / IT;
  const long grid = ntile < spg_num_cus() ? ntile : spg_num_cus();
  return (size_t)grid * CO * CI <= spg_wgrad_workspace_floats(g.M, CO, CI);
}

template <int CO, int CI, int AMODE>
static int launch_bwdpair_t(const SpgBwdPairParams& p, int grid, hipStream_t stream) {
  static bool attr_done = false;
  const size_t lds = spg_bwdpair_lds_bytes<CO, CI>();
  if (!attr_done) {
    hipError_t e = hipFuncSetAttribute(reinterpret_cast<const void*>(&spg_bwdpair_kernel<CO, CI, AMODE>), hipFuncAttributeMaxDynamicSharedMemorySize, (int)lds);
    if (e != hipSuccess) { spg_set_error("hipFuncSetAttribute: %s", hipGetErrorString(e)); return (int)e; }
    attr_done = true;
  }
  hipLaunchKernelGGL((spg_bwdpair_kernel<CO, CI, AMODE>), dim3(grid), dim3(SPG_PAIR_THREADS), lds, stream, p);
  SPG_LAUNCH_CHECK();
  return 0;
}
template <int AMODE>
static int launch_bwdpair_shape(const SpgBwdPairParams& p, int grid, hipStream_t stream) {
  if (p.g.N == 64 && p.g.K == 64) return launch_bwdpair_t<64, 64, AMODE>(p, grid, stream);
  if (p.g.N == 64) return launch_bwdpair_t<128, 64, AMODE>(p, grid, stream);
  return launch_bwdpair_t<128, 128, AMODE>(p, grid, stream);
}

int spg_queue_bwdpair(SpgReduceQueue& q, SpgGemmParams g, const SpgOperand& b, float* dW, hipStream_t stream) {
  SPG_CHECK_ARG(spg_bwdpair_supported(g, b), "shape not supported by the fused backward");
  const int IT = spg_bwdpair_rows(g.N);
  const int ntile = g.M / IT;
  const int grid = ntile < spg_num_cus() ? ntile : spg_num_cus();
  g.ntile = ntile; g.vec_store = 1; g.rows_per_tile = IT;
  const int npass = g.K == 256 ? 2 : 1, COh = g.K / npass;
  for (int h = 0; h < npass; ++h) {
    SpgBwdPairParams p;
    memset(&p, 0, sizeof(p));
    p.g = g; p.b = b;
    p.pass = npass == 1 ? 0 : h + 1;
    if (npass == 2) {
      p.g.K = COh;
      p.g.W = g.W + (long)h * COh * g.ldw;
      p.g.a.X += h * COh; p.g.a.X2 += h * COh;
      if (p.g.a.aidx != nullptr) p.g.a.aidx += h * COh;
      p.g.a.c0 += h * COh; p.g.a.c1 += h * COh; p.g.a.c2 += h * COh; p.g.a.c3 += h * COh;
      if (h == 1) memset(&p.g.fold_bwd, 0, sizeof(p.g.fold_bwd));
    }
    float* dWh = dW + (long)h * COh * g.N;
    if (q.njobs + 1 > SPG_MAX_REDUCE_JOBS) SPG_TRY(spg_flush_reduce(q, stream));
    float* part = dWh;
    if (grid > 1) SPG_TRY(queue_take(q, (size_t)grid * COh * g.N, &part, stream));
    p.partial = part;
    {
      const double flops = 4.0 * (double)g.M * (double)COh * (double)g.N;
      ProfScope prof(stream, flops, SPG_PROF_TAG(4, 64, 64, g.a.mode, SPG_PRO_AFFINE, 1));
      prof.r.M = g.M; prof.r.N = g.N; prof.r.K = COh;
      if (g.a.mode == SPG_PRO_BNBWD) SPG_TRY(launch_bwdpair_shape<SPG_PRO_BNBWD>(p, grid, stream));
      else SPG_TRY(launch_bwdpair_shape<SPG_PRO_POOLBWD>(p, grid, stream));
    }
    if (grid > 1) {
      SpgReduceJob& j = q.jobs[q.njobs++];
      j.partial = part; j.out = dWh; j.nsplit = grid; j.n = COh * g.N;
    }
  }
  SPG_TRY(spg_slot_sync_after(g.stat_slots, spg_fold_slot_words(g.n_mask), stream, false));
  return 0;
}

#define SPG_FIN_SLICES 8

static int* g_fin_counters[SPG_MAX_DEVICES] = {nullptr};
static unsigned g_fin_next[SPG_MAX_DEVICES] = {0};
static std::mutex g_fin_mutex;

static int* spg_fin_counter_window(int n) {
  int dev = 0;
  if (hipGetDevice(&dev) != hipSuccess || dev < 0 || dev >= SPG_MAX_DEVICES) return nullptr;
  std::lock_guard<std::mutex> lock(g_fin_mutex);
  if (g_fin_counters[dev] == nullptr) {
    if (hipMalloc((void**)&g_fin_counters[dev], 4096 * sizeof(int)) != hipSuccess) return nullptr;
    if (hipMemset(g_fin_counters[dev], 0, 4096 * sizeof(int)) != hipSuccess) return nullptr;
  }
  if (g_fin_next[dev] + n > 4096) g_fin_next[dev] = 0;
  int* w = g_fin_counters[dev] + g_fin_next[dev];
  g_fin_next[dev] += n;
  return w;
}

struct SpgBnChannel { float gamma, beta, rm, rv; };
__device__ __forceinline__ SpgBnChannel spg_bn_channel(int c, const float* __restrict__ gamma, const float* __restrict__ beta,
                                                       const float* running_mean, const float* running_var) {
  SpgBnChannel ch;
  ch.gamma = gamma ? gamma[c] : 1.f; ch.beta = beta ? beta[c] : 0.f;
  ch.rm = running_mean ? running_mean[c] : 0.f; ch.rv = running_mean ? running_var[c] : 0.f;
  return ch;
}

__device__ __forceinline__ void spg_bn_finish(double a0, double a1, double a2, double M, int c, const SpgBnChannel& ch,
                                              float* running_mean, float* running_var, float momentum, float eps,
                                              int update_times, float* mean_o, float* rstd_o, float* s_o, float* t_o) {
  const double mean = a0 / M;
  double m2 = a2 + a1 - M * mean * mean;
  if (m2 < 0.0) m2 = 0.0;
  const double var = m2 / M;
  const double rstd = 1.0 / sqrt(var + (double)eps);
  const double g = (double)ch.gamma, be = (double)ch.beta;
  mean_o[c] = (float)mean;
  rstd_o[c] = (float)rstd;
  s_o[c] = (float)(g * rstd);
  t_o[c] = (float)(be - mean * g * rstd);
  if (running_mean != nullptr && update_times > 0) {
    const double uvar = M > 1.0 ? m2 / (M - 1.0) : var;
    float rm = ch.rm, rv = ch.rv;
    for (int u = 0; u < update_times; ++u) {
      rm = (1.f - momentum) * rm + momentum * (float)mean;
      rv = (1.f - momentum) * rv + momentum * (float)uvar;
    }
    running_mean[c] = rm;
    running_var[c] = rv;
  }
}

struct SpgSyncBn {
  spg_allreduce_fn fn = nullptr;
  void* ctx = nullptr;
  double* buf = nullptr;
  long ndoubles = 0;
};
static SpgSyncBn g_sync;

extern "C" int spg_set_bn_allreduce(spg_allreduce_fn fn, void* ctx, double* buf, long buf_doubles) {
  if (fn != nullptr) {
    SPG_CHECK_ARG(buf != nullptr && buf_doubles >= 4, "synchronised BatchNorm needs a device buffer");
    SPG_CHECK_ARG(!spg_slot_sync_active(), "the finalize-based synchronised BatchNorm and the slot-synchronised mode (spg_set_slot_allreduce) exclude each other");
  }
  g_sync.fn = fn; g_sync.ctx = ctx; g_sync.buf = fn ? buf : nullptr; g_sync.ndoubles = fn ? buf_doubles : 0;
  return 0;
}

bool spg_sync_bn_active() { return g_sync.fn != nullptr; }

static int spg_sync_allreduce(long n, hipStream_t stream) {
  const int rc = g_sync.fn(g_sync.ctx, g_sync.buf, n, (void*)stream);
  if (rc != 0) { spg_set_error("the registered BatchNorm all-reduce failed (rc %d)", rc); return -1; }
  return 0;
}

struct SpgSlotSync { spg_slot_allreduce_fn fn = nullptr; void* ctx = nullptr; int world = 1; };
static SpgSlotSync g_slot_sync;
extern "C" int spg_set_slot_allreduce(spg_slot_allreduce_fn fn, void* ctx, int world) {
  if (fn != nullptr) {
    SPG_CHECK_ARG(world >= 1, "slot-synchronised BatchNorm needs the world size");
    SPG_CHECK_ARG(g_sync.fn == nullptr, "slot-synchronised BatchNorm and the finalize-based mode (spg_set_bn_allreduce) exclude each other");
  }
  g_slot_sync.fn = fn; g_slot_sync.ctx = ctx; g_slot_sync.world = fn ? world : 1;
  return 0;
}
bool spg_slot_sync_active() { return g_slot_sync.fn != nullptr; }
int spg_slot_sync_world() { return g_slot_sync.world; }
static int slot_sync_now(unsigned long long* slots, size_t words, hipStream_t stream) {
  const int rc = g_slot_sync.fn(g_slot_sync.ctx, slots, (long)words, (void*)stream);
  if (rc != 0) { spg_set_error("the registered slot all-reduce failed (rc %d)", rc); return -1; }
  return 0;
}

__global__ __launch_bounds__(1024) void spg_bn_finalize_kernel(const float* __restrict__ stat, const float* __restrict__ cnt,
                                                               int nparts, long M, int N, const float* __restrict__ gamma,
                                                               const float* __restrict__ beta, float* running_mean,
                                                               float* running_var, float momentum, float eps,
                                                               int update_times, float* mean_o, float* rstd_o, float* s_o,
                                                               float* t_o, double* __restrict__ scratch, int* counters,
                                                               double* __restrict__ sync_out) {
  __shared__ double r0[16][17], r1[16][17], r2[16][17];
  __shared__ int s_last;
  const int cx = threadIdx.x & 15, ty = threadIdx.x >> 4;
  const int c = blockIdx.x * 16 + cx;
  const int nslices = gridDim.y, slice = blockIdx.y;
  const int per = (nparts + nslices - 1) / nslices;
  const int b0 = slice * per, b1 = min(nparts, b0 + per);
  SpgBnChannel ch = {1.f, 0.f, 0.f, 0.f};
  if (threadIdx.x < 16 && c < N && sync_out == nullptr) ch = spg_bn_channel(c, gamma, beta, running_mean, running_var);
  double a0 = 0.0, a1 = 0.0, a2 = 0.0;
  if (c < N)
    for (int b = b0 + ty; b < b1; b += 512) {
      float nb[8], mb[8], qb[8];
#pragma unroll
      for (int u = 0; u < 8; ++u) {
        const int bb = b + 64 * u;
        const bool ok = bb < b1;
        const long o = ((long)(ok ? bb : b) * 2) * N + c;
        nb[u] = ok ? cnt[bb] : 0.f;
        mb[u] = stat[o];
        qb[u] = ok ? stat[o + N] : 0.f;
      }
#pragma unroll
      for (int u = 0; u < 8; ++u) {
        a0 += (double)nb[u] * (double)mb[u];
        a1 += (double)nb[u] * (double)mb[u] * (double)mb[u];
        a2 += (double)qb[u];
      }
    }
  a0 += __shfl_xor(a0, 16, 64); a1 += __shfl_xor(a1, 16, 64); a2 += __shfl_xor(a2, 16, 64);
  a0 += __shfl_xor(a0, 32, 64); a1 += __shfl_xor(a1, 32, 64); a2 += __shfl_xor(a2, 32, 64);
  const int wave = threadIdx.x >> 6;
  if ((threadIdx.x & 63) < 16) { r0[wave][cx] = a0; r1[wave][cx] = a1; r2[wave][cx] = a2; }
  __syncthreads();
  if (threadIdx.x < 16) {
    a0 = a1 = a2 = 0.0;
    for (int k = 0; k < 16; ++k) { a0 += r0[k][cx]; a1 += r1[k][cx]; a2 += r2[k][cx]; }
  }
  if (nslices > 1) {
    if (threadIdx.x < 16 && c < N) {
      scratch[((long)slice * 3 + 0) * N + c] = a0;
      scratch[((long)slice * 3 + 1) * N + c] = a1;
      scratch[((long)slice * 3 + 2) * N + c] = a2;
    }
// ... 701 lines not shown
```

### superpoint_graph_amd/csrc/spg_narrow.h

```cpp
#pragma once
#include "spg_gemm.h"

#define SPG_GRAM_MAXF 32
inline size_t spg_gram_slot_words(int nfeat) { const int c = nfeat + 1; return (size_t)SPG_FOLD_SLOTS * 2 * (c * (c + 1) / 2) + 8; }

struct SpgGramParams {
  const float* clouds;
  const float* stnT;
  int B, P, Ctot, nfeat;
  unsigned long long* gram;
};
int spg_launch_cloud_gram(const SpgGramParams& p, hipStream_t stream);

struct SpgNarrowPairParams {
  const float* clouds; const float* stnT;
  int P, Ctot, nfeat, nblk;
  double count;
  const float *W1, *b1;
  float* y1;
  const unsigned long long* gram;
  const float *gamma1, *beta1;
  float *rm1, *rv1;
  float *mean1, *rstd1, *s1, *t1;
  int update_times;
  float momentum, eps;
  const float *W2, *b2;
  float* y2;
  unsigned long long* slots2;
};
bool spg_narrow_pair_supported(int nfeat, int c1, int c2, int P, long M);
int spg_launch_narrow_pair_fwd(const SpgNarrowPairParams& p, hipStream_t stream);

struct SpgFirstConvBwdParams {
  const float* clouds; const float* stnT;
  int B, P, Ctot, nfeat;
  const float* g;
  const float* W1;
  const unsigned long long* gram;
  SpgBnFoldBwd fold;
  float* partial;
  float* dT;
};
bool spg_first_conv_bwd_supported(int nfeat, int c1, int P, long M);
int spg_first_conv_bwd_partials(int B);
int spg_launch_first_conv_bwd(const SpgFirstConvBwdParams& p, hipStream_t stream);
```

### superpoint_graph_amd/csrc/spg_narrow.hip

```cpp
#include "../../include/spg_hip.h"
#include "spg_fold.h"
#include "spg_narrow.h"

#pragma clang fp contract(off)

namespace {

#define SPG_NP_C 64
#define SPG_NP_ST1(ptr, v) __builtin_nontemporal_store((v), (ptr))
#define SPG_NP_ST2(ptr, v) __builtin_nontemporal_store((v), (ptr))
#define SPG_NP_W1LD 33
#define SPG_NP_A_SLOTS (16 * 33)
#define SPG_NP_W2_SLOTS (16 * 65)

__global__ __launch_bounds__(256) void spg_cloud_gram_kernel(const SpgGramParams p) {
  __shared__ float xs[128 * (SPG_GRAM_MAXF + 1)];
  const int g = blockIdx.x, P = p.P, nf = p.nfeat, Cg = nf + 1, tid = threadIdx.x;
  const float* base = p.clouds + (long)g * p.Ctot * P;
  for (int i = tid; i < nf * P; i += 256) {
    const int c = i / P, pt = i - c * P;
    xs[pt * Cg + c] = base[i];
  }
  for (int pt = tid; pt < P; pt += 256) xs[pt * Cg + nf] = 1.f;
  __syncthreads();
  if (p.stnT != nullptr) {
    const float* T = p.stnT + (long)g * 4;
    const float t0 = T[0], t1 = T[1], t2 = T[2], t3 = T[3];
    for (int pt = tid; pt < P; pt += 256) {
      const float x = xs[pt * Cg], y = xs[pt * Cg + 1];
      xs[pt * Cg] = fmaf(x, t0 + 1.f, y * t2);
      xs[pt * Cg + 1] = fmaf(x, t1, y * (t3 + 1.f));
    }
    __syncthreads();
  }
  const int npairs = Cg * (Cg + 1) / 2;
  if (blockIdx.x == 0 && tid == 0)
    __hip_atomic_fetch_add(p.gram + (size_t)SPG_FOLD_SLOTS * 2 * npairs + 1, (unsigned long long)((long)p.B * P), __ATOMIC_RELAXED, __HIP_MEMORY_SCOPE_AGENT);
  unsigned long long* slot = p.gram + (size_t)(blockIdx.x & (SPG_FOLD_SLOTS - 1)) * 2 * npairs;
  for (int pr = tid; pr < npairs; pr += 256) {
    int i = 0, rem = pr;
    while (rem >= Cg - i) { rem -= Cg - i; ++i; }
    const int j = i + rem;
    double acc = 0.0;
    for (int pt = 0; pt < P; ++pt) acc = fma((double)xs[pt * Cg + i], (double)xs[pt * Cg + j], acc);
    if (!(fabs(acc) <= 0x1p52)) atomicOr(p.gram + (size_t)SPG_FOLD_SLOTS * 2 * npairs, 1ull);
    long long hi, lo;
    spg_fx_split<-8>(acc, hi, lo);
    __hip_atomic_fetch_add(slot + pr, (unsigned long long)hi, __ATOMIC_RELAXED, __HIP_MEMORY_SCOPE_AGENT);
    __hip_atomic_fetch_add(slot + npairs + pr, (unsigned long long)lo, __ATOMIC_RELAXED, __HIP_MEMORY_SCOPE_AGENT);
  }
}

__device__ __forceinline__ double spg_shfl_xor_d(double v, int m) {
  int lo = __double2loint(v), hi = __double2hiint(v);
  lo = __shfl_xor(lo, m, 64); hi = __shfl_xor(hi, m, 64);
  return __hiloint2double(hi, lo);
}

__device__ __forceinline__ float spg_lane_xor1(float v) {
  return __int_as_float(__builtin_amdgcn_update_dpp(0, __float_as_int(v), 0xB1, 0xF, 0xF, false));
}

typedef double f64x4 __attribute__((ext_vector_type(4)));
#define SPG_GRAM16_SPW 2
__global__ __launch_bounds__(256) void spg_cloud_gram16_kernel(const SpgGramParams p) {
  __shared__ double red[3 * 256];
  const int lane = threadIdx.x & 63, wave = threadIdx.x >> 6;
  const int i = lane & 15, kq = lane >> 4, nf = p.nfeat, P = p.P, Cg = nf + 1;
  f64x4 acc = {0.0, 0.0, 0.0, 0.0};
  const int g0 = __builtin_amdgcn_readfirstlane(((int)blockIdx.x * 4 + wave) * SPG_GRAM16_SPW);
  f32x4 x[SPG_GRAM16_SPW][8], T[SPG_GRAM16_SPW];
#pragma unroll
  for (int q = 0; q < SPG_GRAM16_SPW; ++q) {
    const int g = g0 + q < p.B ? g0 + q : p.B - 1;
    const float* row = p.clouds + ((long)g * p.Ctot + (i < nf ? i : 0)) * P + 4 * kq;
#pragma unroll
    for (int u = 0; u < 8; ++u) {
      x[q][u] = f32x4{0.f, 0.f, 0.f, 0.f};
      if (16 * u < P) x[q][u] = *reinterpret_cast<const f32x4*>(row + 16 * u);
    }
    T[q] = f32x4{0.f, 0.f, 0.f, 0.f};
    if (p.stnT != nullptr) T[q] = *reinterpret_cast<const f32x4*>(p.stnT + (long)g * 4);
  }
#pragma unroll
  for (int q = 0; q < SPG_GRAM16_SPW; ++q) {
    if (g0 + q >= p.B) break;
#pragma unroll
    for (int u = 0; u < 8; ++u) {
      if (16 * u >= P) break;
#pragma unroll
      for (int e = 0; e < 4; ++e) {
        float v = x[q][u][e];
        if (p.stnT != nullptr) {
          const float other = spg_lane_xor1(v);
          if (i == 0) v = fmaf(v, T[q][0] + 1.f, other * T[q][2]);
          else if (i == 1) v = fmaf(other, T[q][1], v * (T[q][3] + 1.f));
        }
        v = i < nf ? v : (i == nf ? 1.f : 0.f);
        const double d = (double)v;
        acc = __builtin_amdgcn_mfma_f64_16x16x4f64(d, d, acc, 0, 0, 0);
      }
    }
  }
  if (wave > 0) {
#pragma unroll
    for (int v = 0; v < 4; ++v) red[(wave - 1) * 256 + v * 64 + lane] = acc[v];
  }
  __syncthreads();
  if (wave != 0) return;
#pragma unroll
  for (int w = 0; w < 3; ++w)
#pragma unroll
    for (int v = 0; v < 4; ++v) acc[v] += red[w * 256 + v * 64 + lane];
  const int npairs = Cg * (Cg + 1) / 2;
  if (blockIdx.x == 0 && lane == 0)
    __hip_atomic_fetch_add(p.gram + (size_t)SPG_FOLD_SLOTS * 2 * npairs + 1, (unsigned long long)((long)p.B * P), __ATOMIC_RELAXED, __HIP_MEMORY_SCOPE_AGENT);
  unsigned long long* slot = p.gram + (size_t)(blockIdx.x & (SPG_FOLD_SLOTS - 1)) * 2 * npairs;
  const int j = lane & 15;
#pragma unroll
  for (int v = 0; v < 4; ++v) {
    const int ii = (lane >> 4) + 4 * v;
    if (ii <= j && j < Cg) {
      const int pr = ii * Cg - ii * (ii - 1) / 2 + (j - ii);
      const double a = acc[v];
      if (!(fabs(a) <= 0x1p52)) atomicOr(p.gram + (size_t)SPG_FOLD_SLOTS * 2 * npairs, 1ull);
      long long hi, lo;
      spg_fx_split<-8>(a, hi, lo);
      __hip_atomic_fetch_add(slot + pr, (unsigned long long)hi, __ATOMIC_RELAXED, __HIP_MEMORY_SCOPE_AGENT);
      __hip_atomic_fetch_add(slot + npairs + pr, (unsigned long long)lo, __ATOMIC_RELAXED, __HIP_MEMORY_SCOPE_AGENT);
    }
  }
}

template <int KG>
__device__ __forceinline__ void spg_np_load_x(const SpgNarrowPairParams& p, int blk, int bps, int r, int h, float (&v)[4 * KG], f32x4& T) {
  const int g = blk / bps, p0 = (blk - g * bps) * 32;
  const unsigned xo = (unsigned)(g * p.Ctot * p.P + p0 + r);
#pragma unroll
  for (int gq = 0; gq < KG; ++gq)
#pragma unroll
    for (int s = 0; s < 4; ++s) {
      const int c = 8 * gq + 4 * h + s;
      const float t = p.clouds[xo + (unsigned)((c < p.nfeat ? c : 0) * p.P)];
      v[gq * 4 + s] = c < p.nfeat ? t : 0.f;
    }
  T = f32x4{0.f, 0.f, 0.f, 0.f};
  if (p.stnT != nullptr) T = *reinterpret_cast<const f32x4*>(p.stnT + (long)g * 4);
}

template <int KG, int NW>
__global__ __launch_bounds__(64 * NW) void spg_narrow_pair_fwd_kernel(const SpgNarrowPairParams p) {
  extern __shared__ f32x4 smem[];
  f32x4* W2s = smem;
  float* W1s = reinterpret_cast<float*>(smem + SPG_NP_W2_SLOTS + NW * SPG_NP_A_SLOTS);
  float* cst = W1s + SPG_NP_C * SPG_NP_W1LD;
// ... 286 lines not shown
  if (blockIdx.x + 1 == gridDim.x) {
    const bool bad = p.gram[(size_t)SPG_FOLD_SLOTS * 2 * npairs] != 0ull;
    for (int pr = tid; pr < npairs; pr += NT) {
      int i = 0, rem = pr;
      while (rem >= Cg - i) { rem -= Cg - i; ++i; }
      const int j = i + rem;
      double g = spg_fx_sum<-8>(p.gram + pr, (size_t)npairs, (size_t)2 * npairs);
      if (bad) g = __builtin_nan("");
      Gs[i * Cg + j] = g;
      Gs[j * Cg + i] = g;
    }
    __syncthreads();
    float* out = p.partial + (size_t)((int)gridDim.x - 1) * (SPG_NP_C * nf);
    for (int e = tid; e < SPG_NP_C * nf; e += NT) {
      const int c = e / nf, k = e - c * nf;
      const double xk = Gs[k * Cg + nf] / M;
      double a = 0.0;
#pragma unroll 1
      for (int jj = 0; jj < nf; ++jj) a = fma((double)p.W1[(long)c * nf + jj], Gs[jj * Cg + k] - Gs[jj * Cg + nf] * xk, a);
      out[e] = (float)(-(double)cs[3 * SPG_NP_C + c] * a * (p.fold.grad_mul > 0.0 ? p.fold.grad_mul : 1.0));
    }
    return;
  }
  {
    const int part = tid & 7, nout = 2 * nf + 2;
    for (int o0 = 0; o0 < nout; o0 += NT / 8) {
      const int o = o0 + (tid >> 3);
      double a = 0.0;
      if (o < nout) {
        const bool isk2 = o >= 2 * nf;
        const int n = isk2 ? o - 2 * nf : o / nf, k = isk2 ? 0 : o - n * nf;
        for (int c = part; c < SPG_NP_C; c += 8) {
          const double wn = (double)p.W1[(long)c * nf + n];
          a = isk2 ? fma((double)cs[c] * (double)cs[SPG_NP_C + c], wn, a) : fma((double)p.W1[(long)c * nf + k] * (double)cs[3 * SPG_NP_C + c], wn, a);
        }
      }
      a += spg_shfl_xor_d(a, 4); a += spg_shfl_xor_d(a, 2); a += spg_shfl_xor_d(a, 1);
      if (o < nout && part == 0) {
        if (o >= 2 * nf) k2[o - 2 * nf] = (float)a; else vn[o / nf][o - (o / nf) * nf] = (float)a;
      }
    }
  }
  __syncthreads();

  float un[2][2], vl[2];
#pragma unroll
  for (int n = 0; n < 2; ++n) {
    un[n][0] = cs[r] * w1n[0][n];
    un[n][1] = cs[r + 32] * w1n[1][n];
    vl[n] = r < nf ? vn[n][r] : 0.f;
  }
  const float xbl = r < nf ? xbar[r] : 0.f;
  const float k2l = k2[r >> 4];
  const int total = ((int)gridDim.x - 1) * NW;
  f32x16 acc[2];
#pragma unroll
  for (int j = 0; j < 2; ++j)
#pragma unroll
    for (int q = 0; q < 16; ++q) acc[j][q] = 0.f;

#pragma unroll 1
  for (int g = (int)blockIdx.x * NW + wave; g < p.B; g += total) {
    float gvS[BPS][16][2], xrS[BPS][2];
    f32x4 x4S[BPS][4];
    const float* xc = p.clouds + ((long)g * p.Ctot + (r < nf ? r : 0)) * P + 4 * h;
#pragma unroll
    for (int b = 0; b < BPS; ++b) {
      const float* gb = p.g + ((long)g * P + 32 * b) * SPG_NP_C + r;
#pragma unroll
      for (int t = 0; t < 16; ++t)
#pragma unroll
        for (int j = 0; j < 2; ++j) gvS[b][t][j] = gb[spg_fcb_row(t, h) * SPG_NP_C + 32 * j];
#pragma unroll
      for (int q = 0; q < 4; ++q) x4S[b][q] = *reinterpret_cast<const f32x4*>(xc + 32 * b + 8 * q);
      xrS[b][0] = 0.f; xrS[b][1] = 0.f;
      if (WANT_DT) {
        const float* rb = p.clouds + ((long)g * p.Ctot) * P + 32 * b + spg_fcb_row(r & 15, h);
        xrS[b][0] = rb[0]; xrS[b][1] = rb[P];
      }
    }
    f32x4 T = f32x4{0.f, 0.f, 0.f, 0.f};
    if (p.stnT != nullptr) T = *reinterpret_cast<const f32x4*>(p.stnT + (long)g * 4);
    float dta0 = 0.f, dta1 = 0.f;
#pragma unroll
    for (int b = 0; b < BPS; ++b) {
      float (&gv)[16][2] = gvS[b];
      float xa[16];
#pragma unroll
      for (int t = 0; t < 16; ++t) {
        float v = x4S[b][t >> 2][t & 3];
        if (p.stnT != nullptr) {
          const float other = spg_lane_xor1(v);
          const float tx = fmaf(v, T[0] + 1.f, other * T[2]), ty = fmaf(other, T[1], v * (T[3] + 1.f));
          v = r == 0 ? tx : (r == 1 ? ty : v);
        }
        xa[t] = r < nf ? v - xbl : 0.f;
      }
#pragma unroll
      for (int t = 0; t < 16; ++t)
#pragma unroll
        for (int j = 0; j < 2; ++j) acc[j] = __builtin_amdgcn_mfma_f32_32x32x2f32(xa[t], gv[t][j], acc[j], 0, 0, 0);
      if (WANT_DT) {
        float dxy = 0.f;
#pragma unroll
        for (int n = 0; n < 2; ++n) {
          float V[16];
#pragma unroll
          for (int t = 0; t < 16; ++t) V[t] = fmaf(gv[t][0], un[n][0], fmaf(gv[t][1], un[n][1], -(xa[t] * vl[n])));
#pragma unroll
          for (int m = 8; m >= 1; m >>= 1) {
            const bool up = (r & m) != 0;
#pragma unroll
            for (int i = 0; i < m; ++i) {
              float lo_ = V[i], hi_ = V[i + m];
              asm volatile("" : "+v"(lo_), "+v"(hi_));
              const float send = up ? lo_ : hi_, keep = up ? hi_ : lo_;
              V[i] = keep + __shfl_xor(send, m, 64);
            }
          }
          const float tot = V[0] + __shfl_xor(V[0], 16, 64);
          if ((r >> 4) == n) dxy = tot - k2l;
        }
        dta0 = fmaf(xrS[b][0], dxy, dta0);
        dta1 = fmaf(xrS[b][1], dxy, dta1);
      }
    }
    if (WANT_DT) {
      const float a00 = spg_wave_sum(r < 16 ? dta0 : 0.f), a01 = spg_wave_sum(r < 16 ? 0.f : dta0);
      const float a10 = spg_wave_sum(r < 16 ? dta1 : 0.f), a11 = spg_wave_sum(r < 16 ? 0.f : dta1);
      if (lane == 0) { float* o = p.dT + (long)g * 4; o[0] = a00; o[1] = a01; o[2] = a10; o[3] = a11; }
    }
  }
  {
    extern __shared__ float red[];
#pragma unroll
    for (int j = 0; j < 2; ++j)
#pragma unroll
      for (int q = 0; q < 16; ++q) red[(wave * 32 + j * 16 + q) * 64 + lane] = acc[j][q];
    __syncthreads();
    float* out = p.partial + (size_t)blockIdx.x * (SPG_NP_C * nf);
    for (int e = tid; e < 32 * 64; e += NT) {
      const int jq = e >> 6, l = e & 63, j = jq >> 4, q = jq & 15;
      const int k = spg_acc_row(q, l >> 5), c = (l & 31) + 32 * j;
      if (k < nf) {
        float a = red[e];
#pragma unroll
        for (int w = 1; w < NW; ++w) a += red[w * 32 * 64 + e];
        out[c * nf + k] = cs[c] * a;
      }
    }
  }
}

}

bool spg_narrow_pair_supported(int nfeat, int c1, int c2, int P, long M) {
  return nfeat >= 1 && nfeat <= SPG_GRAM_MAXF && c1 == SPG_NP_C && c2 == SPG_NP_C && P >= 32 && P <= 128 && P % 32 == 0 && M > 0 &&
         M * SPG_NP_C * 4 < (1L << 32) && M * (long)nfeat * 4 < (1L << 32) && spg_tune_get(SPG_TUNE_NO_NARROW_PAIR) != 1;
}

int spg_launch_cloud_gram(const SpgGramParams& p, hipStream_t stream) {
  SPG_CHECK_ARG(p.clouds && p.gram && p.B > 0 && p.P >= 1 && p.P <= 128 && p.nfeat >= 1 && p.nfeat <= SPG_GRAM_MAXF, "gram arguments");
  if (p.nfeat + 1 <= 16 && p.P % 16 == 0 && spg_tune_get(SPG_TUNE_NO_NARROW_PAIR) != 2)
    hipLaunchKernelGGL(spg_cloud_gram16_kernel, dim3(spg_cdiv(p.B, 4 * SPG_GRAM16_SPW)), dim3(256), 0, stream, p);
  else
    hipLaunchKernelGGL(spg_cloud_gram_kernel, dim3(p.B), dim3(256), 0, stream, p);
  SPG_LAUNCH_CHECK();
  return 0;
}

int spg_launch_narrow_pair_fwd(const SpgNarrowPairParams& p, hipStream_t stream) {
  SPG_CHECK_ARG(p.clouds && p.W1 && p.W2 && p.y1 && p.y2 && p.gram && p.slots2 && p.mean1 && p.rstd1 && p.s1 && p.t1, "null pointer");
  SPG_CHECK_ARG(p.P % 32 == 0 && p.nblk > 0 && p.count > 0.0, "blocks of 32 points");
  SpgProfSpan prof(stream, 2.0 * p.count * SPG_NP_C * (p.nfeat + SPG_NP_C), 5000000 + 1, SPG_NP_C, SPG_NP_C);
  return p.nfeat <= 16 ? launch_pair<2>(p, stream) : launch_pair<4>(p, stream);
}

bool spg_first_conv_bwd_supported(int nfeat, int c1, int P, long M) {
  return nfeat >= 2 && nfeat <= SPG_GRAM_MAXF && c1 == SPG_NP_C && P >= 32 && P <= 128 && P % 32 == 0 && M > 0 && M * SPG_NP_C * 4 < (1L << 32) &&
         spg_tune_get(SPG_TUNE_NO_NARROW_PAIR) == 0 && !spg_tune_get(SPG_TUNE_NO_FIRST_CONV_BWD);
}

static int fcb_grid(int B) {
  int dev = 0, cus = 256;
  if (hipGetDevice(&dev) != hipSuccess || hipDeviceGetAttribute(&cus, hipDeviceAttributeMultiprocessorCount, dev) != hipSuccess || cus <= 0) cus = 256;
  const int need = spg_cdiv(B, SPG_FCB_NW);
  return need < 2 * cus ? need : 2 * cus;
}
int spg_first_conv_bwd_partials(int B) { return fcb_grid(B) + 1; }

int spg_launch_first_conv_bwd(const SpgFirstConvBwdParams& p, hipStream_t stream) {
  SPG_CHECK_ARG(p.clouds && p.g && p.W1 && p.gram && p.partial && p.fold.slots && p.fold.consts && p.fold.C == SPG_NP_C, "first-convolution backward arguments");
  const int grid = fcb_grid(p.B);
  SpgProfSpan prof(stream, 2.0 * (double)p.B * p.P * SPG_NP_C * (p.nfeat + (p.dT != nullptr ? 2 : 0)), 5000000 + 2, SPG_NP_C, p.nfeat);
  const size_t lds = (size_t)SPG_FCB_NW * 32 * 64 * sizeof(float);
  const dim3 gd(grid + 1), bd(64 * SPG_FCB_NW);
#define SPG_FCB_LAUNCH(DT, BPS_) hipLaunchKernelGGL((spg_first_conv_bwd_kernel<DT, BPS_>), gd, bd, lds, stream, p)
  const int bps = p.P / 32;
  if (p.dT != nullptr) { if (bps == 1) SPG_FCB_LAUNCH(true, 1); else if (bps == 2) SPG_FCB_LAUNCH(true, 2); else if (bps == 3) SPG_FCB_LAUNCH(true, 3); else SPG_FCB_LAUNCH(true, 4); }
  else { if (bps == 1) SPG_FCB_LAUNCH(false, 1); else if (bps == 2) SPG_FCB_LAUNCH(false, 2); else if (bps == 3) SPG_FCB_LAUNCH(false, 3); else SPG_FCB_LAUNCH(false, 4); }
#undef SPG_FCB_LAUNCH
  SPG_LAUNCH_CHECK();
  return 0;
}
```

### superpoint_graph_amd/csrc/spg_pointnet.hip

```cpp
#include "../../include/spg_hip.h"
#include "spg_ecc.h"
#include "spg_gemm.h"
#include "spg_narrow.h"
#include <limits.h>
#include <mutex>
#include <unordered_map>
#include <vector>

namespace {
std::mutex g_gram_mu;
std::unordered_map<const void*, bool> g_gram_filled;
void gram_record(const void* slots, bool filled) { std::lock_guard<std::mutex> lock(g_gram_mu); g_gram_filled[slots] = filled; }
bool gram_recorded(const void* slots) {
  std::lock_guard<std::mutex> lock(g_gram_mu);
  auto it = g_gram_filled.find(slots);
  return it != g_gram_filled.end() && it->second;
}

struct Layer {
  int cin = 0, cout = 0;
  bool bn = false;
  bool conv = false;
  const float *W = nullptr, *b = nullptr, *gamma = nullptr, *beta = nullptr;
  float *rm = nullptr, *rv = nullptr;
// ... 179 lines not shown
  if (!is_fc) {
    if (k == 0) return op_cloud(pl, clouds, stnT);
    const Layer& p = pl.L[sg.convs[k - 1]];
    return op_affine(p, p.y, p.ldy, p.cout);
  }
  if (k == 0) {
    const Layer& p = pl.L[sg.convs.back()];
    return op_affine(p, sg.pooled, sg.ldpool, p.cout);
  }
  const Layer& p = pl.L[sg.fcs[k - 1]];
  return op_affine(p, p.y, p.ldy, p.cout);
}

SpgBnFold fold_of(const Plan& pl, const Layer& prod, long count, int update_times) {
  SpgBnFold f; memset(&f, 0, sizeof(f));
  if (!pl.fold || !prod.bn) return f;
  f.slots = prod.slots; f.C = prod.cout; f.update_times = update_times; f.momentum = pl.cfg.bn_momentum; f.eps = pl.cfg.bn_eps;
  f.count = (double)count; f.gamma = prod.gamma; f.beta = prod.beta; f.rm = prod.rm; f.rv = prod.rv;
  f.mean = prod.mean; f.rstd = prod.rstd; f.s = prod.s; f.t = prod.t;
  return f;
}

int bn_stats(const Plan& pl, Layer& l, int nparts, long M, int update_times, hipStream_t st) {
  if (pl.training && pl.fold) return 0;
  if (pl.training)
    return spg_launch_bn_finalize(pl.stat, pl.stat_cnt, nparts, M, l.cout, l.gamma, l.beta, l.rm, l.rv,
                                  pl.cfg.bn_momentum, pl.cfg.bn_eps, update_times, l.mean, l.rstd, l.s, l.t, pl.fin, st);
  return 0;
}

bool fused_eval_convs(Plan& pl, Segment& sg, const float* clouds, const float* stnT, SpgConvStackParams& cp) {
  if (pl.training || sg.convs.size() > SPG_CONVSTACK_MAX_LAYERS) return false;
  memset(&cp, 0, sizeof(cp));
  cp.clouds = clouds; cp.stnT = stnT; cp.B = pl.B; cp.P = pl.P; cp.Ctot = pl.cfg.nfeat; cp.nlayers = (int)sg.convs.size();
  for (size_t k = 0; k < sg.convs.size(); ++k) {
    const Layer& l = pl.L[sg.convs[k]];
    if (!l.bn) return false;
    cp.cin[k] = l.cin; cp.cout[k] = l.cout; cp.W[k] = l.W; cp.bias[k] = l.b; cp.s[k] = l.s; cp.t[k] = l.t;
    cp.Wp[k] = reinterpret_cast<f32x4*>(l.Wpack);
  }
  cp.pmax = pl.pmax; cp.pmin = pl.pmin;
  return spg_conv_stack_eval_supported(cp);
}

int forward_segment(Plan& pl, Segment& sg, const float* clouds, const float* stnT, int update_times, hipStream_t st) {
  SpgConvStackParams cp;
  const bool fused = fused_eval_convs(pl, sg, clouds, stnT, cp);
  if (fused) {
    const Layer& ll = pl.L[sg.convs.back()];
    SPG_TRY(spg_launch_conv_stack_eval(cp, st));
    SPG_TRY(spg_launch_pool_select_parts(pl.pmax, pl.pmin, nullptr, nullptr, ll.s, pl.B, ll.cout, 4, sg.extra, sg.nextra,
                                         sg.pooled, sg.ldpool, nullptr, st));
  }
  size_t kfirst = 0;
  if (pl.training && sg.gram != nullptr) gram_record(sg.gram, false);
  if (!fused && pl.training && pl.fold && sg.gram != nullptr && sg.convs.size() > 2) {
    Layer& l0 = pl.L[sg.convs[0]];
    Layer& l1 = pl.L[sg.convs[1]];
    if (l0.bn && l1.bn && spg_narrow_pair_supported(l0.cin, l0.cout, l1.cout, pl.P, pl.M)) {
      SpgGramParams gp; memset(&gp, 0, sizeof(gp));
      gp.clouds = clouds; gp.stnT = stnT; gp.B = pl.B; gp.P = pl.P; gp.Ctot = pl.cfg.nfeat; gp.nfeat = l0.cin; gp.gram = sg.gram;
      SPG_TRY(spg_launch_cloud_gram(gp, st));
      SPG_TRY(spg_slot_sync_after(sg.gram, spg_gram_slot_words(l0.cin), st, false));
      SpgNarrowPairParams np; memset(&np, 0, sizeof(np));
      np.clouds = clouds; np.stnT = stnT; np.P = pl.P; np.Ctot = pl.cfg.nfeat; np.nfeat = l0.cin; np.nblk = (int)(pl.M / 32);
      np.count = (double)pl.M;
      np.W1 = l0.W; np.b1 = l0.b; np.y1 = l0.y; np.gram = sg.gram; np.gamma1 = l0.gamma; np.beta1 = l0.beta; np.rm1 = l0.rm; np.rv1 = l0.rv;
      np.mean1 = l0.mean; np.rstd1 = l0.rstd; np.s1 = l0.s; np.t1 = l0.t;
      np.update_times = update_times; np.momentum = pl.cfg.bn_momentum; np.eps = pl.cfg.bn_eps;
      np.W2 = l1.W; np.b2 = l1.b; np.y2 = l1.y; np.slots2 = l1.slots;
      SPG_TRY(spg_launch_narrow_pair_fwd(np, st));
      SPG_TRY(spg_slot_sync_after(l1.slots, spg_fold_slot_words(l1.cout), st, false));
      gram_record(sg.gram, true);
      kfirst = 2;
    }
  }
  for (size_t k = kfirst; !fused && k < sg.convs.size(); ++k) {
    Layer& l = pl.L[sg.convs[k]];
    const bool last = k + 1 == sg.convs.size();
    SpgGemmParams g; memset(&g, 0, sizeof(g));
    g.a = input_operand(pl, sg, false, k, clouds, stnT);
    if (k > 0) g.fold = fold_of(pl, pl.L[sg.convs[k - 1]], pl.M, update_times);
    g.W = l.W; g.ldw = l.cin; g.bias = l.b; g.M = (int)pl.M; g.N = l.cout; g.K = l.cin;
    g.rows_per_tile = pl.P; g.epi = SPG_EPI_FWD; g.Y = l.y; g.ldy = l.ldy;
    if (l.Wb_f != nullptr) { g.Wb = l.Wb_f; g.ldwb = spg_split_ld(l.cin); g.wb_part_bytes = (long)l.cout * g.ldwb * 2; }
    if (last && !pl.training) g.Y = nullptr;
    g.stat = pl.training ? pl.stat : nullptr; g.stat_cnt = pl.stat_cnt;
    if (pl.fold) { g.stat = nullptr; g.stat_slots = l.slots; }
    int nparts = 0;
    if (last) {
      g.pool_out = sg.pooled; g.pool_idx = sg.aidx; g.pool_ld = sg.ldpool; g.pool_sign = l.gamma;
      g.pool_extra = sg.extra; g.pool_nextra = sg.nextra;
    }
    SPG_TRY(spg_launch_gemm(g, st, &nparts));
    SPG_TRY(bn_stats(pl, l, nparts, pl.M, update_times, st));
  }
  SpgGroupScope grp(st);
  for (size_t k = 0; k < sg.fcs.size(); ++k) {
    Layer& l = pl.L[sg.fcs[k]];
    SpgGemmParams g; memset(&g, 0, sizeof(g));
    g.a = input_operand(pl, sg, true, k, clouds, stnT);
    g.fold = k == 0 ? fold_of(pl, pl.L[sg.convs.back()], pl.M, update_times) : fold_of(pl, pl.L[sg.fcs[k - 1]], pl.B, update_times);
    if (!pl.pads_done) {
      bool mine = false;
      for (int idx : sg.fcs) mine = mine || pl.L[idx].Wpad != nullptr;
      if (mine && k == 0) {
        for (Layer& q : pl.L) if (q.Wpad) SPG_TRY(spg_launch_pad_rows(q.W, q.cin, q.Wpad, q.ldw, q.cout, q.cin, st));
        SPG_TRY(grp.flush());
      } else if (!mine) {
        for (Layer& q : pl.L) if (q.Wpad) SPG_TRY(spg_launch_pad_rows(q.W, q.cin, q.Wpad, q.ldw, q.cout, q.cin, st));
      }
      pl.pads_done = true;
    }
    g.W = l.Wpad ? l.Wpad : l.W; g.ldw = l.ldw; g.bias = l.b; g.M = pl.B; g.N = l.cout; g.K = l.cin;
    g.rows_per_tile = SPG_FC_ROWS; g.epi = SPG_EPI_FWD; g.Y = l.y; g.ldy = l.ldy;
    g.stat = (pl.training && l.bn) ? pl.stat : nullptr; g.stat_cnt = pl.stat_cnt;
    if (pl.fold && l.bn) { g.stat = nullptr; g.stat_slots = l.slots; }
    int nparts = 0;
    {
      SpgGroupBypass direct(l.bn && pl.training && !pl.fold);
      SPG_TRY(spg_launch_gemm(g, st, &nparts));
    }
    SPG_TRY(grp.flush());
    if (l.bn) SPG_TRY(bn_stats(pl, l, nparts, pl.B, update_times, st));
  }
  return 0;
}

struct BwdScratch {
  float *dzA = nullptr, *dzB = nullptr;
  float *fzA = nullptr, *fzB = nullptr;
  float* consts = nullptr;
  double* fin = nullptr;
  float* work = nullptr;
  size_t work_floats = 0;
  float* stat = nullptr;
  float* dxy = nullptr;
  float* dT = nullptr;
  float* grad_global = nullptr;
  size_t bytes = 0;
};

void carve_bwd(const Plan& pl, void* ws, BwdScratch& s) {
  Carver cv(ws);
  int cconv = 4, cfc = 4, cmax = 4;
  size_t wmax = 16, workmax = 16;
  for (const Layer& l : pl.L) {
    if (l.conv) { cconv = l.cin > cconv ? l.cin : cconv; }
    else { cfc = l.cin + 4 > cfc ? l.cin + 4 : cfc; }
    cmax = l.cout > cmax ? l.cout : cmax; cmax = l.cin > cmax ? l.cin : cmax;
    wmax = (size_t)l.cin * l.cout > wmax ? (size_t)l.cin * l.cout : wmax;
    workmax += ((spg_wgrad_workspace_floats(l.conv ? pl.M : pl.B, l.cout, l.cin) + 63) & ~(size_t)63) + 64 * (size_t)l.cout + 128 +
               ((spg_wgrad_colsum_floats(l.conv ? pl.M : pl.B, l.cout, l.cin) + 63) & ~(size_t)63);
    if (l.conv && l.cin <= SPG_GRAM_MAXF) workmax += ((size_t)spg_first_conv_bwd_partials(pl.B) * l.cout * l.cin + 63) & ~(size_t)63;
  }
  s.dzA = cv.take<float>((size_t)pl.M * cconv); s.dzB = cv.take<float>((size_t)pl.M * cconv);
  s.fzA = cv.take<float>((size_t)pl.B * cfc); s.fzB = cv.take<float>((size_t)pl.B * cfc);
  s.consts = cv.take<float>((size_t)4 * cmax);
  s.fin = cv.take<double>(spg_bn_finalize_scratch_doubles(cmax));
  s.work = cv.take<float>(workmax); s.work_floats = workmax;
  s.stat = cv.take<float>((size_t)pl.B * 4 * 2 * cmax);
  s.dxy = cv.take<float>((size_t)pl.M * 2);
  s.dT = cv.take<float>((size_t)pl.B * 4);
  s.bytes = cv.off + 256;
}

SpgOperand op_bnbwd(const float* dz, const float* y, long ld, const float* consts, int C) {
  SpgOperand o; memset(&o, 0, sizeof(o));
  o.mode = SPG_PRO_BNBWD; o.X = dz; o.X2 = y; o.ld = ld;
  o.c0 = consts; o.c1 = consts + C; o.c2 = consts + 2 * C; o.c3 = consts + 3 * C;
  return o;
}

int zero_async(float* p, size_t n, hipStream_t st) {
  if (p == nullptr || n == 0) return 0;
  hipError_t e = hipMemsetAsync(p, 0, n * sizeof(float), st);
  if (e != hipSuccess) { spg_set_error("hipMemsetAsync: %s", hipGetErrorString(e)); return (int)e; }
  return 0;
}

SpgBnFoldBwd fold_bwd_of(const Plan& pl, const Layer& prod, long count, float* consts) {
  SpgBnFoldBwd f; memset(&f, 0, sizeof(f));
  f.slots = prod.slots_bwd; f.C = prod.cout; f.count = (double)count; f.s = prod.s; f.mean = prod.mean; f.rstd = prod.rstd;
  f.consts = consts; f.dgamma = prod.dgamma; f.dbeta = prod.dbeta;
  if (spg_slot_sync_active()) f.grad_mul = 1.0 / (double)spg_slot_sync_world();
  return f;
}

int backward_segment(Plan& pl, Segment& sg, BwdScratch& s, SpgReduceQueue& rq, SpgOperand cur, const float* clouds,
                     const float* stnT, bool want_dxy, hipStream_t st, bool ride_reduce = false,
                     float* dT_out = nullptr, bool* dT_done = nullptr) {
  const int B = pl.B;
  SpgBnFoldBwd pending; memset(&pending, 0, sizeof(pending));
  float* fz[2] = {s.fzA, s.fzB};
  int flip = 0;
  {
  SpgGroupScope grp(st);
  for (int k = (int)sg.fcs.size() - 1; k >= 0; --k) {
    if (ride_reduce) SPG_TRY(spg_reduce_ride(rq, st));
    Layer& l = pl.L[sg.fcs[k]];
    SpgWgradParams w; memset(&w, 0, sizeof(w));
    w.a = cur; w.b = input_operand(pl, sg, true, k, clouds, stnT); w.M = B; w.N = l.cout; w.K = l.cin;
    w.fold = pending;
    const SpgBnFoldBwd fold_k = pending;
    memset(&pending, 0, sizeof(pending));
    const bool bias_rides = l.db != nullptr && !l.bn && cur.mode == SPG_PRO_IDENT;
    SPG_TRY(spg_queue_wgrad(rq, w, l.dW, st, bias_rides ? l.db : nullptr));
    if (l.db && !bias_rides) {
      if (l.bn) SPG_TRY(spg_group_zero(l.db, l.cout, st));
      else SPG_TRY(spg_queue_colsum(rq, cur.X, cur.ld, B, l.cout, l.db, st));
    }
    const bool first = k == 0;
    Layer& prod = first ? pl.L[sg.convs.back()] : pl.L[sg.fcs[k - 1]];
    float* out = fz[flip]; flip ^= 1;
    SpgGemmParams g; memset(&g, 0, sizeof(g));
    g.a = cur; g.W = l.Wpad ? l.Wpad : l.W; g.ldw = l.ldw; g.w_red = 1;
    g.M = B; g.N = l.cin; g.K = l.cout; g.rows_per_tile = SPG_FC_ROWS;
    g.epi = SPG_EPI_BWD; g.Y = out; g.ldy = first ? sg.ldpool : l.cin;
    g.Yp = first ? sg.pooled : prod.y; g.ldyp = first ? sg.ldpool : prod.ldy;
    g.ms = prod.s; g.mt = prod.t; g.mask_relu = 1; g.n_mask = prod.cout;
    g.mmean = prod.mean; g.mrstd = prod.rstd; g.stat = s.stat;
    if (pl.fold) { g.stat = nullptr; g.stat_slots = prod.slots_bwd; g.stat_rows = first ? pl.M : (long)B; }
    if (grp.active()) g.fold_bwd = fold_k;
    int nparts = 0;
    SPG_TRY(spg_launch_gemm(g, st, &nparts));
    SPG_TRY(grp.flush());
    const int C = prod.cout;
    if (first && s.grad_global != nullptr && sg.nextra > 0)
      SPG_TRY(spg_launch_copy2d(out + C, sg.ldpool, s.grad_global, sg.nextra, B, sg.nextra, st));
    if (pl.fold) pending = fold_bwd_of(pl, prod, first ? pl.M : (long)B, s.consts);
    else
    SPG_TRY(spg_launch_bn_bwd_finalize(s.stat, nparts, l.cin, first ? pl.M : (long)B, C, prod.s, prod.mean,
                                       prod.rstd, s.consts, prod.dgamma, prod.dbeta, s.fin, st));
    if (!first) {
      cur = op_bnbwd(out, prod.y, prod.ldy, s.consts, C);
    } else {
      memset(&cur, 0, sizeof(cur));
      cur.mode = SPG_PRO_POOLBWD; cur.X = out; cur.ldg = (int)sg.ldpool; cur.aidx = sg.aidx; cur.P = pl.P;
      cur.X2 = prod.y; cur.ld = prod.ldy;
      cur.c0 = s.consts; cur.c1 = s.consts + C; cur.c2 = s.consts + 2 * C; cur.c3 = s.consts + 3 * C;
    }
  }
  }
  float* dz[2] = {s.dzA, s.dzB};
  flip = 0;
  for (int k = (int)sg.convs.size() - 1; k >= 0; --k) {
    Layer& l = pl.L[sg.convs[k]];
    if (k > 0 && pl.fold) {
      Layer& prod = pl.L[sg.convs[k - 1]];
      float* out = dz[flip];
      SpgGemmParams g; memset(&g, 0, sizeof(g));
      g.a = cur; g.W = l.W; g.ldw = l.cin; g.w_red = 1;
      g.M = (int)pl.M; g.N = l.cin; g.K = l.cout; g.rows_per_tile = pl.P;
      g.epi = SPG_EPI_BWD; g.Y = out; g.ldy = l.cin; g.Yp = prod.y; g.ldyp = prod.ldy;
      g.ms = prod.s; g.mt = prod.t; g.mask_relu = 1; g.n_mask = prod.cout;
      g.mmean = prod.mean; g.mrstd = prod.rstd; g.stat_slots = prod.slots_bwd; g.fold_bwd = pending;
      const SpgOperand xin = input_operand(pl, sg, false, k, clouds, stnT);
      if (spg_bwdpair_supported(g, xin)) {
        SPG_TRY(spg_queue_bwdpair(rq, g, xin, l.dW, st));
        if (l.db) SPG_TRY(zero_async(l.db, l.cout, st));
        flip ^= 1;
        pending = fold_bwd_of(pl, prod, pl.M, s.consts);
        cur = op_bnbwd(out, prod.y, prod.ldy, s.consts, prod.cout);
        continue;
      }
    }
    if (k == 0 && pl.fold && sg.gram != nullptr && gram_recorded(sg.gram) && sg.convs.size() > 2 && pending.slots != nullptr && cur.mode == SPG_PRO_BNBWD &&
        cur.ld == l.cout && cur.c0 == s.consts && (!want_dxy || dT_out != nullptr) &&
        spg_narrow_pair_supported(l.cin, l.cout, pl.L[sg.convs[1]].cout, pl.P, pl.M) && spg_first_conv_bwd_supported(l.cin, l.cout, pl.P, pl.M)) {
      SpgFirstConvBwdParams fp; memset(&fp, 0, sizeof(fp));
      fp.clouds = clouds; fp.stnT = stnT; fp.B = pl.B; fp.P = pl.P; fp.Ctot = pl.cfg.nfeat; fp.nfeat = l.cin;
      fp.g = cur.X; fp.W1 = l.W; fp.gram = sg.gram; fp.fold = pending; memset(&pending, 0, sizeof(pending));
      fp.dT = want_dxy ? dT_out : nullptr;
      SPG_TRY(spg_queue_partials(rq, spg_first_conv_bwd_partials(pl.B), l.cout * l.cin, l.dW, &fp.partial, st));
      SPG_TRY(spg_launch_first_conv_bwd(fp, st));
      if (l.db) SPG_TRY(zero_async(l.db, l.cout, st));
      if (want_dxy && dT_done != nullptr) *dT_done = true;
      continue;
    }
    SpgWgradParams w; memset(&w, 0, sizeof(w));
    w.a = cur; w.b = input_operand(pl, sg, false, k, clouds, stnT); w.M = (int)pl.M; w.N = l.cout; w.K = l.cin;
    w.fold = pending; memset(&pending, 0, sizeof(pending));
    w.allow_lowp = 1;
    SPG_TRY(spg_queue_wgrad(rq, w, l.dW, st));
    if (l.db) SPG_TRY(zero_async(l.db, l.cout, st));
    if (k > 0) {
      Layer& prod = pl.L[sg.convs[k - 1]];
      float* out = dz[flip]; flip ^= 1;
      SpgGemmParams g; memset(&g, 0, sizeof(g));
      g.a = cur; g.W = l.W; g.ldw = l.cin; g.w_red = 1;
      g.M = (int)pl.M; g.N = l.cin; g.K = l.cout; g.rows_per_tile = pl.P;
      if (l.Wb_t != nullptr) { g.Wb = l.Wb_t; g.ldwb = spg_split_ld(l.cout); g.wb_part_bytes = (long)l.cin * g.ldwb * 2; }
      g.epi = SPG_EPI_BWD; g.Y = out; g.ldy = l.cin; g.Yp = prod.y; g.ldyp = prod.ldy;
      g.ms = prod.s; g.mt = prod.t; g.mask_relu = 1; g.n_mask = prod.cout;
      g.mmean = prod.mean; g.mrstd = prod.rstd; g.stat = s.stat;
      const bool foldk = pl.fold && !spg_gemm_bwd_stats_want_partials(g);
      if (foldk) { g.stat = nullptr; g.stat_slots = prod.slots_bwd; }
      int nparts = 0;
      SPG_TRY(spg_launch_gemm(g, st, &nparts));
      if (foldk) pending = fold_bwd_of(pl, prod, pl.M, s.consts);
      else
      SPG_TRY(spg_launch_bn_bwd_finalize(s.stat, nparts, l.cin, pl.M, prod.cout, prod.s, prod.mean, prod.rstd, s.consts,
                                         prod.dgamma, prod.dbeta, s.fin, st));
      cur = op_bnbwd(out, prod.y, prod.ldy, s.consts, prod.cout);
    } else if (want_dxy) {
      SpgGemmParams g; memset(&g, 0, sizeof(g));
      g.a = cur; g.W = l.Wpad ? l.Wpad : l.W; g.ldw = l.Wpad ? l.ldw : l.cin; g.w_red = 1;
      g.M = (int)pl.M; g.N = 2; g.K = l.cout; g.rows_per_tile = pl.P;
      g.epi = SPG_EPI_BWD; g.Y = s.dxy; g.ldy = 2;
      SPG_TRY(spg_launch_gemm(g, st));
    }
  }
  return 0;
}

void bind_grads(Plan& pl, void* const* grads) {
  for (size_t i = 0; i < pl.L.size(); ++i) {
    void* const* g = grads + 6 * i;
    pl.L[i].dW = (float*)g[0]; pl.L[i].db = (float*)g[1]; pl.L[i].dgamma = (float*)g[2]; pl.L[i].dbeta = (float*)g[3];
  }
}

}

extern "C" int spg_pointnet_num_layers(const spg_pointnet_cfg* cfg) { return cfg ? num_layers(*cfg) : -1; }

extern "C" size_t spg_pointnet_workspace_bytes(const spg_pointnet_cfg* cfg, int B, int training) {
  Plan pl;
  if (make_plan(cfg, B, training, nullptr, nullptr, nullptr, pl) != 0) return 0;
  return pl.bytes;
}

extern "C" int spg_pointnet_forward(const spg_pointnet_cfg* cfg, int B, const float* clouds, const float* clouds_global,
                                    const void* const* params, float* emb, void* workspace, int training,
                                    int bn_update_times, void* stream) {
  return spg_pointnet_forward_ext(cfg, B, clouds, clouds_global, nullptr, params, emb, workspace, training, bn_update_times, stream);
}

static thread_local bool g_slots_clean = false, g_slots_clear_at_end = false;
void spg_pointnet_set_step_flags(bool clean, bool clear_at_end) { g_slots_clean = clean; g_slots_clear_at_end = clear_at_end; }

extern "C" int spg_pointnet_forward_ext(const spg_pointnet_cfg* cfg, int B, const float* clouds, const float* clouds_global,
                                        const float* ext_transform, const void* const* params, float* emb, void* workspace,
                                        int training, int bn_update_times, void* stream) {
  SPG_CHECK_ARG(clouds && params && emb && workspace, "null pointer");
  SPG_CHECK_ARG(ext_transform == nullptr || cfg->nfeat_stn == 0, "an external transform replaces the inner STN (nfeat_stn must be 0)");
  hipStream_t st = (hipStream_t)stream;
  Plan pl;
  SPG_TRY(make_plan(cfg, B, training, workspace, params, emb, pl));
  SPG_CHECK_ARG(pl.cfg.nfeat_global == 0 || clouds_global != nullptr, "clouds_global is required");
  pl.main.extra = clouds_global;
  if (!pl.training) {
    SpgBnEvalBatch eb;
    for (Layer& l : pl.L)
      if (l.bn) {
        SPG_CHECK_ARG(eb.njobs < SPG_BN_EVAL_MAX_JOBS, "too many BatchNorm layers");
        eb.jobs[eb.njobs++] = SpgBnEvalJob{l.cout, l.gamma, l.beta, l.rm, l.rv, l.s, l.t};
      }
    SPG_TRY(spg_launch_bn_eval_batch(eb, pl.cfg.bn_eps, st));
  }
  if (pl.training && spg_gemm_precision() != 0) {
    SpgSplitBatch sb;
    for (Layer& l : pl.L)
      if (l.Wb_f != nullptr) {
        SPG_CHECK_ARG(sb.njobs < SPG_SPLIT_MAX_JOBS, "too many layers");
        sb.jobs[sb.njobs++] = SpgSplitJob{l.W, l.cin, l.cout, l.cin, l.Wb_f, l.Wb_t};
      }
    SPG_TRY(spg_launch_split_weights(sb, st));
  }
  pl.fold = pl.training && !spg_sync_bn_active() && !spg_tune_get(SPG_TUNE_NO_BN_FOLD) && 4L * B * spg_slot_sync_world() <= SPG_FOLD_MAX_CONTRIBUTIONS;
  SPG_CHECK_ARG(!(pl.training && spg_slot_sync_active()) || pl.fold, "slot-synchronised BatchNorm needs the statistics slots (spg_tune key 10 off, batch within the slots' capacity)");
  if (pl.training && !g_slots_clean) {
    hipError_t me = hipMemsetAsync(pl.slots_all, 0, pl.slots_words * sizeof(unsigned long long), st);
    if (me != hipSuccess) { spg_set_error("hipMemsetAsync: %s", hipGetErrorString(me)); return (int)me; }
  }
  const float* stnT = ext_transform;
  if (pl.has_stn) {
    SPG_TRY(forward_segment(pl, pl.stn, clouds, nullptr, bn_update_times, st));
    stnT = pl.L[pl.stn.fcs.back()].y;
  }
  SPG_TRY(forward_segment(pl, pl.main, clouds, stnT, bn_update_times, st));
  return 0;
}

extern "C" long spg_pointnet_debug_offset(const spg_pointnet_cfg* cfg, int B, int training, int layer, int what) {
  Plan pl;
  char* fake = (char*)(uintptr_t)4096;
  if (make_plan(cfg, B, training, fake, nullptr, (float*)(uintptr_t)8, pl) != 0) return -1;
  const void* p = nullptr;
  if (layer == -1 || layer == -2) {
    const Segment& sg = layer == -1 ? pl.stn : pl.main;
    if (layer == -1 && !pl.has_stn) return -1;
    if (what == 2) return sg.ldpool;
    p = what == 1 ? (const void*)sg.aidx : (const void*)sg.pooled;
  }
  else if (layer >= 0 && layer < (int)pl.L.size()) {
    const Layer& l = pl.L[layer];
    p = what == 0 ? (const void*)l.y : what == 1 ? l.s : what == 2 ? l.t : what == 3 ? l.mean : l.rstd;
    if (what == 0 && l.y == (float*)(uintptr_t)8) return -1;
  }
  if (p == nullptr) return -1;
  return (long)((const char*)p - fake);
}

extern "C" size_t spg_pointnet_bwd_workspace_bytes(const spg_pointnet_cfg* cfg, int B) {
  Plan pl;
  if (make_plan(cfg, B, 1, nullptr, nullptr, nullptr, pl) != 0) return 0;
  BwdScratch s;
  carve_bwd(pl, nullptr, s);
  return s.bytes;
}

extern "C" int spg_pointnet_backward(const spg_pointnet_cfg* cfg, int B, const float* clouds, const float* clouds_global,
                                     const void* const* params, const float* grad_emb, void* const* grads,
                                     void* workspace, void* bwd_workspace, void* stream) {
  return spg_pointnet_backward_ext(cfg, B, clouds, clouds_global, nullptr, params, grad_emb, grads, nullptr, nullptr, workspace,
                                   bwd_workspace, stream);
}
// ... 41 lines not shown
```

Before: 925,800 superpoints/s.

## Fuse first-conv weight-gradient contraction into the 64x64 backward pair kernel

Adds an FC variant of the fused backward pair kernel. While the kernel computes the layer-1 input gradient, it stages that gradient tile in LDS and contracts it against the (STN-transformed, mean-centred) cloud features with MFMA, producing first-layer weight-gradient partials or per-tile q blocks. A new lightweight finish kernel then folds BN terms and produces dW1 and dT. This replaces the separate first-conv backward pass, which re-read the layer-1 gradient from global memory. The cost is extra LDS, extra work in the pair kernel, and more complex coupling between the two layers.

```diff
diff --git a/include/spg_hip.h b/include/spg_hip.h
--- a/include/spg_hip.h
+++ b/include/spg_hip.h
@@ -223,6 +223,7 @@
 int spg_prof_tag(int kind, int it, int jt, int x, int y, int full);
 int spg_prof_read_shapes(int* keys, double* vals, int max);
 int spg_tune(int key, int value);
+long spg_first_conv_fused_launches(int reset);
 typedef struct spg_step_args {
   const spg_pointnet_cfg* ptn_cfg;
   int B, bn_update_times;
diff --git a/superpoint_graph_amd/_lib.py b/superpoint_graph_amd/_lib.py
--- a/superpoint_graph_amd/_lib.py
+++ b/superpoint_graph_amd/_lib.py
@@ -164,6 +164,7 @@
     'spg_prof_read_tag': (_i, [_i, ctypes.POINTER(ctypes.c_double), ctypes.POINTER(ctypes.c_long), ctypes.POINTER(ctypes.c_double)]),
     'spg_prof_read_shapes': (_i, [ctypes.POINTER(_i), ctypes.POINTER(ctypes.c_double), _i]),
     'spg_tune': (_i, [_i, _i]),
+    'spg_first_conv_fused_launches': (_l, [_i]),
     'spg_prof_read': (_i, [ctypes.POINTER(ctypes.c_double), ctypes.POINTER(ctypes.c_long), ctypes.POINTER(ctypes.c_double), _i]),
 }
 
diff --git a/superpoint_graph_amd/csrc/spg_common.h b/superpoint_graph_amd/csrc/spg_common.h
--- a/superpoint_graph_amd/csrc/spg_common.h
+++ b/superpoint_graph_amd/csrc/spg_common.h
@@ -15,7 +15,7 @@
 extern "C" const char* spg_last_error(void);
 void spg_set_error(const char* fmt, ...);
 enum { SPG_TUNE_NO_PERSIST = 0, SPG_TUNE_DBG = 3, SPG_TUNE_FIN_SLICE_MIN = 4, SPG_TUNE_NO_STAT_ACCUM = 5, SPG_TUNE_NO_HEAD_SERVICE = 6, SPG_TUNE_PRECISION = 7,
-       SPG_TUNE_NO_PERSIST_ECC = 8, SPG_TUNE_NO_BN_FOLD = 10, SPG_TUNE_NO_GROUP = 11, SPG_TUNE_NO_BWD_PAIR = 14, SPG_TUNE_NO_ECC_HEAD = 15, SPG_TUNE_NO_NARROW_PAIR = 17, SPG_TUNE_NO_FIRST_CONV_BWD = 18, SPG_TUNE_PX_SPIN_LIMIT = 20, SPG_TUNE_NO_ADAM_GUARD = 21, SPG_TUNE_NO_PAIR_SPLIT = 22, SPG_TUNE_COUNT = 23 };
+       SPG_TUNE_NO_PERSIST_ECC = 8, SPG_TUNE_NO_BN_FOLD = 10, SPG_TUNE_NO_GROUP = 11, SPG_TUNE_NO_BWD_PAIR = 14, SPG_TUNE_NO_ECC_HEAD = 15, SPG_TUNE_NO_NARROW_PAIR = 17, SPG_TUNE_NO_FIRST_CONV_BWD = 18, SPG_TUNE_PX_SPIN_LIMIT = 20, SPG_TUNE_NO_ADAM_GUARD = 21, SPG_TUNE_NO_PAIR_SPLIT = 22, SPG_TUNE_NO_FIRST_CONV_FUSED = 23, SPG_TUNE_COUNT = 24 };
 int spg_tune_get(int key);
 
 #define SPG_CHECK_ARG(cond, msg)                                          \
diff --git a/superpoint_graph_amd/csrc/spg_gemm.h b/superpoint_graph_amd/csrc/spg_gemm.h
--- a/superpoint_graph_amd/csrc/spg_gemm.h
+++ b/superpoint_graph_amd/csrc/spg_gemm.h
@@ -146,7 +146,18 @@
 };
 int spg_queue_wgrad(SpgReduceQueue& q, SpgWgradParams p, float* dW, hipStream_t stream, float* db = nullptr);
 bool spg_bwdpair_supported(const SpgGemmParams& g, const SpgOperand& b);
-int spg_queue_bwdpair(SpgReduceQueue& q, SpgGemmParams g, const SpgOperand& b, float* dW, hipStream_t stream);
+struct SpgPairFirstConv {
+  const float* clouds; const float* stnT;
+  const unsigned long long* gram;
+  int P, Ctot, nfeat, per_tile;
+  double rows;
+  float* q;
+  float* dW1;
+  int nparts;
+};
+bool spg_bwdpair_first_conv_supported(const SpgGemmParams& g, const SpgPairFirstConv& fc);
+int spg_bwdpair_grid(long M, int CI);
+int spg_queue_bwdpair(SpgReduceQueue& q, SpgGemmParams g, const SpgOperand& b, float* dW, hipStream_t stream, SpgPairFirstConv* fc = nullptr);
 int spg_queue_partials(SpgReduceQueue& q, int nsplit, int n, float* out, float** partial, hipStream_t stream);
 int spg_queue_colsum(SpgReduceQueue& q, const float* X, long ld, long M, int N, float* out, hipStream_t stream);
 int spg_flush_reduce(SpgReduceQueue& q, hipStream_t stream);
diff --git a/superpoint_graph_amd/csrc/spg_gemm.hip b/superpoint_graph_amd/csrc/spg_gemm.hip
--- a/superpoint_graph_amd/csrc/spg_gemm.hip
+++ b/superpoint_graph_amd/csrc/spg_gemm.hip
@@ -61,6 +61,7 @@
 #ifndef SPG_ATTRIBUTION
   if ((key == SPG_TUNE_DBG || key == SPG_TUNE_NO_STAT_ACCUM) && value != 0) return -1;
 #endif
+  if (key == SPG_TUNE_NO_FIRST_CONV_FUSED && value != 0 && value != 1) return -1;
   const int old = g_tune[key];
   g_tune[key] = value;
   return old;
@@ -1688,10 +1689,11 @@
   return 0;
 }
 
-template <int IT, int JT, int WI, int WJ>
+#define SPG_PAIR_GQ_LD 68
+template <int IT, int JT, int WI, int WJ, bool FC = false>
 __device__ __forceinline__ void spg_epilogue_bwd_vec_lds(const SpgGemmParams& p, f32x16 (&acc)[IT / WI / 32][JT / WJ / 32],
                                                          float* __restrict__ red, const float* __restrict__ ylds, int ldl, long m0,
-                                                         SpgStatAcc<JT / WJ / 32>& sacc, const int pass) {
+                                                         SpgStatAcc<JT / WJ / 32>& sacc, const int pass, float* __restrict__ gq = nullptr) {
   constexpr int TI = IT / WI / 32, TJ = JT / WJ / 32, RW = IT / WI, CW = JT / WJ;
   constexpr int LD = CW + 8, LPR = CW / 4, RPI = 64 / LPR, NIT = SPG_EPI_PIECE_ROWS / RPI;
   const int tid = threadIdx.x + spg_opaque_zero(), lane = tid & 63, wave = (tid >> 6) & 3;
@@ -1739,6 +1741,8 @@
           s1 += v;
           s2 = spg_fma4(v, xhat, s2);
         }
+        if constexpr (FC) *reinterpret_cast<f32x4*>(gq + (roww + rb + lr + RPI * u) * SPG_PAIR_GQ_LD + col) = v;
+        else
         __builtin_nontemporal_store(v, reinterpret_cast<f32x4*>(yo + oo0 + (unsigned)(rb + RPI * u) * (unsigned)p.ldy));
       }
       __builtin_amdgcn_sched_barrier(0);
@@ -1752,6 +1756,7 @@
   float* partial;
   int pass;
   int pad_;
+  SpgPairFirstConv fc;
 };
 #define SPG_PAIR_THREADS 1024
 #ifdef SPG_ATTRIBUTION
@@ -1781,13 +1786,14 @@
 #define SPG_TP(k)
 #define SPG_TEND(role)
 #endif
-template <int CO, int CI>
+template <int CO, int CI, bool FC = false>
 constexpr size_t spg_bwdpair_lds_bytes() {
   return 2 * ((size_t)(CO / 4) * (spg_bwdpair_rows(CI) + 1) * 16 + (size_t)spg_bwdpair_rows(CI) * (CI + 4) * 4) + (size_t)CO * (CI + 4) * 4 +
-         (size_t)4 * SPG_EPI_WAVE_FLOATS(32, 32) * 4 + (size_t)(CO + CI / 2) * 16;
-}
-
-template <int CO, int CI, int AMODE>
+         (size_t)4 * SPG_EPI_WAVE_FLOATS(32, 32) * 4 + (size_t)(CO + CI / 2) * 16 +
+         (FC ? (size_t)2 * spg_bwdpair_rows(CI) * SPG_PAIR_GQ_LD * 4 : 0);
+}
+
+template <int CO, int CI, int AMODE, bool FC = false>
 __global__ __launch_bounds__(SPG_PAIR_THREADS) void spg_bwdpair_kernel(const SpgBwdPairParams p) {
   constexpr int IT = spg_bwdpair_rows(CI), SA = IT + 1, SX = CI + 4;
   constexpr int CQ = CO / 4, XQ = CI / 4;
@@ -1804,6 +1810,8 @@
   float* wl = reinterpret_cast<float*>(smem + 2 * BUF4);
   float* red = wl + CO * SX;
   f32x4* kst = reinterpret_cast<f32x4*>(red + 4 * SPG_EPI_WAVE_FLOATS(32, 32));
+  float* gqs = reinterpret_cast<float*>(kst + CO + CI / 2);
+  static_assert(!FC || (CO == 64 && CI == 64), "the first-layer contraction rides in the 64 -> 64 pair");
   const SpgGemmParams& g = p.g;
   const int tid = threadIdx.x, lane = tid & 63;
   const int wave = __builtin_amdgcn_readfirstlane(tid >> 6);
@@ -1935,6 +1943,16 @@
     return;
   }
 
+  [[maybe_unused]] float fc_xbar = 0.f;
+  [[maybe_unused]] const int fc_n = lane & 15, fc_s = lane >> 4;
+  if constexpr (FC) {
+    if (role == 0 && fc_n < p.fc.nfeat) {
+      const int nf = p.fc.nfeat, Cg = nf + 1, npairs = Cg * (Cg + 1) / 2, pr = fc_n * Cg - fc_n * (fc_n - 1) / 2 + (nf - fc_n);
+      const unsigned long long nrow = p.fc.gram[(size_t)SPG_FOLD_SLOTS * 2 * npairs + 1];
+      const double Mg = nrow != 0ull ? (double)nrow : p.fc.rows;
+      fc_xbar = (float)(spg_fx_sum<-8>(p.fc.gram + pr, (size_t)npairs, (size_t)2 * npairs) / Mg);
+    }
+  }
   prologue(std::true_type{});
   if (role == 0) {
     f32x16 acc[1][1];
@@ -1944,21 +1962,72 @@
     __syncthreads();
     SPG_TQ(3); SPG_TQEND();
     int buf = 0;
+    [[maybe_unused]] f32x4 fc_acc = {0.f, 0.f, 0.f, 0.f}, fc_u[4], fc_T = {0.f, 0.f, 0.f, 0.f};
+    [[maybe_unused]] int fc_pend = -1;
+    [[maybe_unused]] const int fc_w = wave & 3;
+    [[maybe_unused]] auto fc_load = [&](int t) __attribute__((always_inline)) {
+      const int nf = p.fc.nfeat, P = p.fc.P;
+      const int row0 = t * IT, b = row0 / P, p0 = row0 - b * P;
+      const int ch = fc_n < nf ? fc_n : (fc_n >= 14 ? fc_n - 14 : 0);
+      const float* xc = p.fc.clouds + ((long)b * p.fc.Ctot + ch) * P + p0 + 4 * fc_s;
+#pragma unroll
+      for (int q = 0; q < 4; ++q) fc_u[q] = *reinterpret_cast<const f32x4*>(xc + 16 * q);
+      if (p.fc.stnT != nullptr) fc_T = *reinterpret_cast<const f32x4*>(p.fc.stnT + (long)b * 4);
+    };
+    [[maybe_unused]] auto fc_contract = [&](int t, int gbuf) __attribute__((always_inline)) {
+      const float* gt = gqs + gbuf * (IT * SPG_PAIR_GQ_LD) + 4 * fc_s * SPG_PAIR_GQ_LD + 16 * fc_w + fc_n;
+      const bool centred = fc_n < p.fc.nfeat, raw = fc_n >= 14 && p.fc.per_tile != 0;
+      if (p.fc.per_tile) fc_acc = f32x4{0.f, 0.f, 0.f, 0.f};
+#pragma unroll
+      for (int q = 0; q < 4; ++q)
+#pragma unroll
+        for (int j = 0; j < 4; ++j) {
+          float v = fc_u[q][j];
+          if (p.fc.stnT != nullptr) {
+            const float other = __int_as_float(__builtin_amdgcn_update_dpp(0, __float_as_int(v), 0xB1, 0xF, 0xF, false));
+            const float tx = fmaf(v, fc_T[0] + 1.f, other * fc_T[2]), ty = fmaf(other, fc_T[1], v * (fc_T[3] + 1.f));
+            v = fc_n == 0 ? tx : (fc_n == 1 ? ty : v);
+          }
+          const float u = centred ? v - fc_xbar : (raw ? v : 0.f);
+          fc_acc = __builtin_amdgcn_mfma_f32_16x16x4f32(gt[(16 * q + j) * SPG_PAIR_GQ_LD], u, fc_acc, 0, 0, 0);
+        }
+      if (p.fc.per_tile) {
+        float* qo = p.fc.q + (long)t * (CI * 16) + (16 * fc_w + 4 * fc_s) * 16 + fc_n;
+#pragma unroll
+        for (int e = 0; e < 4; ++e) qo[16 * e] = fc_acc[e];
+      }
+    };
     SPG_T0();
     for (;;) {
       const int nxt = tile + stride;
       const bool has_next = nxt < ntile;
       const f32x4* dz4 = smem + buf * BUF4;
+      if constexpr (FC) { if (fc_pend >= 0) fc_load(fc_pend); }
 #pragma unroll
       for (int q = 0; q < 16; ++q) acc[0][0][q] = 0.f;
       spg_mfma_tile_or<CO / 8, 2>(dz4, wl, SA, SX, wi * 32 + r, wj * 32 + r, h, acc[0][0]);
+      if constexpr (FC) { if (fc_pend >= 0) fc_contract(fc_pend, buf ^ 1); }
       SPG_TP(0);
-      spg_epilogue_bwd_vec_lds<IT, CI, WI, WJ>(g, acc, red, reinterpret_cast<const float*>(dz4 + CQ * SA), SX, (long)tile * IT, sacc, p.pass);
+      spg_epilogue_bwd_vec_lds<IT, CI, WI, WJ, FC>(g, acc, red, reinterpret_cast<const float*>(dz4 + CQ * SA), SX, (long)tile * IT, sacc, p.pass,
+                                                   FC ? gqs + buf * (IT * SPG_PAIR_GQ_LD) : nullptr);
       SPG_TP(1);
       __syncthreads();
       SPG_TP(2);
+      if constexpr (FC) fc_pend = tile;
       if (!has_next) break;
       tile = nxt; buf ^= 1;
+    }
+    if constexpr (FC) {
+      fc_load(fc_pend);
+      fc_contract(fc_pend, buf);
+      if (!p.fc.per_tile && fc_n < p.fc.nfeat) {
+        float* po = p.fc.q + (long)blockIdx.x * (CI * p.fc.nfeat);
+#pragma unroll
+        for (int e = 0; e < 4; ++e) {
+          const int c = 16 * fc_w + 4 * fc_s + e;
+          po[c * p.fc.nfeat + fc_n] = g.ms[c] * fc_acc[e];
+        }
+      }
     }
     SPG_TEND(0);
     if (p.pass == 1) return;
@@ -2045,37 +2114,61 @@
   return (size_t)grid * CO * CI <= spg_wgrad_workspace_floats(g.M, CO, CI);
 }
 
-template <int CO, int CI, int AMODE>
+int spg_bwdpair_grid(long M, int CI) {
+  const long ntile = M / spg_bwdpair_rows(CI);
+  return (int)(ntile < spg_num_cus() ? ntile : spg_num_cus());
+}
+
+bool spg_bwdpair_first_conv_supported(const SpgGemmParams& g, const SpgPairFirstConv& fc) {
+  if (g.N != 64 || g.K != 64 || g.a.mode != SPG_PRO_BNBWD) return false;
+  if (fc.clouds == nullptr || fc.gram == nullptr || fc.P < 64 || fc.P % 64 != 0 || (long)g.M % fc.P != 0) return false;
+  if (fc.nfeat < 2 || fc.nfeat + 2 > 16 || fc.Ctot < fc.nfeat) return false;
+  if ((((uintptr_t)fc.clouds) & 15) != 0 || (fc.stnT != nullptr && (((uintptr_t)fc.stnT) & 15) != 0)) return false;
+  if (fc.per_tile && (fc.q == nullptr || (((uintptr_t)fc.q) & 15) != 0)) return false;
+  if (!fc.per_tile && fc.dW1 == nullptr) return false;
+  return true;
+}
+
+template <int CO, int CI, int AMODE, bool FC = false>
 static int launch_bwdpair_t(const SpgBwdPairParams& p, int grid, hipStream_t stream) {
   static bool attr_done = false;
-  const size_t lds = spg_bwdpair_lds_bytes<CO, CI>();
+  const size_t lds = spg_bwdpair_lds_bytes<CO, CI, FC>();
   if (!attr_done) {
-    hipError_t e = hipFuncSetAttribute(reinterpret_cast<const void*>(&spg_bwdpair_kernel<CO, CI, AMODE>), hipFuncAttributeMaxDynamicSharedMemorySize, (int)lds);
+    hipError_t e = hipFuncSetAttribute(reinterpret_cast<const void*>(&spg_bwdpair_kernel<CO, CI, AMODE, FC>), hipFuncAttributeMaxDynamicSharedMemorySize, (int)lds);
     if (e != hipSuccess) { spg_set_error("hipFuncSetAttribute: %s", hipGetErrorString(e)); return (int)e; }
     attr_done = true;
   }
-  hipLaunchKernelGGL((spg_bwdpair_kernel<CO, CI, AMODE>), dim3(grid), dim3(SPG_PAIR_THREADS), lds, stream, p);
+  hipLaunchKernelGGL((spg_bwdpair_kernel<CO, CI, AMODE, FC>), dim3(grid), dim3(SPG_PAIR_THREADS), lds, stream, p);
   SPG_LAUNCH_CHECK();
   return 0;
 }
 template <int AMODE>
 static int launch_bwdpair_shape(const SpgBwdPairParams& p, int grid, hipStream_t stream) {
+  if constexpr (AMODE == SPG_PRO_BNBWD) {
+    if (p.fc.clouds != nullptr) return launch_bwdpair_t<64, 64, AMODE, true>(p, grid, stream);
+  }
   if (p.g.N == 64 && p.g.K == 64) return launch_bwdpair_t<64, 64, AMODE>(p, grid, stream);
   if (p.g.N == 64) return launch_bwdpair_t<128, 64, AMODE>(p, grid, stream);
   return launch_bwdpair_t<128, 128, AMODE>(p, grid, stream);
 }
 
-int spg_queue_bwdpair(SpgReduceQueue& q, SpgGemmParams g, const SpgOperand& b, float* dW, hipStream_t stream) {
+int spg_queue_bwdpair(SpgReduceQueue& q, SpgGemmParams g, const SpgOperand& b, float* dW, hipStream_t stream, SpgPairFirstConv* fc) {
   SPG_CHECK_ARG(spg_bwdpair_supported(g, b), "shape not supported by the fused backward");
+  SPG_CHECK_ARG(fc == nullptr || spg_bwdpair_first_conv_supported(g, *fc), "first-layer contraction not supported for this pair");
   const int IT = spg_bwdpair_rows(g.N);
   const int ntile = g.M / IT;
   const int grid = ntile < spg_num_cus() ? ntile : spg_num_cus();
+  if (fc != nullptr && !fc->per_tile) {
+    fc->nparts = grid + 1;
+    SPG_TRY(queue_take(q, (size_t)fc->nparts * g.N * fc->nfeat, &fc->q, stream));
+  }
   g.ntile = ntile; g.vec_store = 1; g.rows_per_tile = IT;
   const int npass = g.K == 256 ? 2 : 1, COh = g.K / npass;
   for (int h = 0; h < npass; ++h) {
     SpgBwdPairParams p;
     memset(&p, 0, sizeof(p));
     p.g = g; p.b = b;
+    if (fc != nullptr) p.fc = *fc;
     p.pass = npass == 1 ? 0 : h + 1;
     if (npass == 2) {
       p.g.K = COh;
@@ -2101,6 +2194,11 @@
       SpgReduceJob& j = q.jobs[q.njobs++];
       j.partial = part; j.out = dWh; j.nsplit = grid; j.n = COh * g.N;
     }
+  }
+  if (fc != nullptr && !fc->per_tile) {
+    if (q.njobs + 1 > SPG_MAX_REDUCE_JOBS) SPG_TRY(spg_flush_reduce(q, stream));
+    SpgReduceJob& j = q.jobs[q.njobs++];
+    j.partial = fc->q; j.out = fc->dW1; j.nsplit = fc->nparts; j.n = g.N * fc->nfeat;
   }
   SPG_TRY(spg_slot_sync_after(g.stat_slots, spg_fold_slot_words(g.n_mask), stream, false));
   return 0;
diff --git a/superpoint_graph_amd/csrc/spg_narrow.h b/superpoint_graph_amd/csrc/spg_narrow.h
--- a/superpoint_graph_amd/csrc/spg_narrow.h
+++ b/superpoint_graph_amd/csrc/spg_narrow.h
@@ -44,3 +44,15 @@
 bool spg_first_conv_bwd_supported(int nfeat, int c1, int P, long M);
 int spg_first_conv_bwd_partials(int B);
 int spg_launch_first_conv_bwd(const SpgFirstConvBwdParams& p, hipStream_t stream);
+
+struct SpgFirstConvFinishParams {
+  const float* clouds; const float* stnT;
+  int B, P, Ctot, nfeat;
+  const float* q;
+  const float* W1;
+  const unsigned long long* gram;
+  SpgBnFoldBwd fold;
+  float* partial;
+  float* dT;
+};
+int spg_launch_first_conv_finish(const SpgFirstConvFinishParams& p, hipStream_t stream);
diff --git a/superpoint_graph_amd/csrc/spg_narrow.hip b/superpoint_graph_amd/csrc/spg_narrow.hip
--- a/superpoint_graph_amd/csrc/spg_narrow.hip
+++ b/superpoint_graph_amd/csrc/spg_narrow.hip
@@ -1,6 +1,7 @@
 #include "../../include/spg_hip.h"
 #include "spg_fold.h"
 #include "spg_narrow.h"
+#include <atomic>
 
 #pragma clang fp contract(off)
 
@@ -593,6 +594,131 @@
   }
 }
 
+template <bool PER_SP>
+__global__ __launch_bounds__(64 * SPG_FCB_NW) void spg_first_conv_finish_kernel(const SpgFirstConvFinishParams p) {
+  constexpr int NW = SPG_FCB_NW, NT = 64 * NW;
+  __shared__ double Gs[(SPG_GRAM_MAXF + 1) * (SPG_GRAM_MAXF + 1)];
+  __shared__ float cs[4 * SPG_NP_C];
+  __shared__ float xbar[SPG_GRAM_MAXF + 1];
+  __shared__ float vn[2][SPG_GRAM_MAXF + 1];
+  __shared__ float k2[2];
+  __shared__ float red[PER_SP ? NW * SPG_NP_C * 16 : 1];
+  const int tid = threadIdx.x, lane = tid & 63, wave = __builtin_amdgcn_readfirstlane(tid >> 6);
+  const int nf = p.nfeat, Cg = nf + 1, npairs = Cg * (Cg + 1) / 2, P = p.P;
+  const unsigned long long nrow = p.gram[(size_t)SPG_FOLD_SLOTS * 2 * npairs + 1];
+  const double M = nrow != 0ull ? (double)nrow : (double)p.B * (double)P;
+  float w1n[2] = {0.f, 0.f};
+  if (PER_SP) { w1n[0] = p.W1[(long)lane * nf]; w1n[1] = p.W1[(long)lane * nf + 1]; }
+  if (tid < nf) {
+    const int i = tid, pr = i * Cg - i * (i - 1) / 2 + (nf - i);
+    xbar[tid] = (float)(spg_fx_sum<-8>(p.gram + pr, (size_t)npairs, (size_t)2 * npairs) / M);
+  }
+  spg_bn_fold_bwd(p.fold, blockIdx.x == 0);
+  for (int i = tid; i < 4 * SPG_NP_C; i += NT) cs[i] = p.fold.consts[i];
+  __syncthreads();
+  if (blockIdx.x + 1 == gridDim.x) {
+    const bool bad = p.gram[(size_t)SPG_FOLD_SLOTS * 2 * npairs] != 0ull;
+    for (int pr = tid; pr < npairs; pr += NT) {
+      int i = 0, rem = pr;
+      while (rem >= Cg - i) { rem -= Cg - i; ++i; }
+      const int j = i + rem;
+      double g = spg_fx_sum<-8>(p.gram + pr, (size_t)npairs, (size_t)2 * npairs);
+      if (bad) g = __builtin_nan("");
+      Gs[i * Cg + j] = g;
+      Gs[j * Cg + i] = g;
+    }
+    __syncthreads();
+    float* out = p.partial + (PER_SP ? (size_t)((int)gridDim.x - 1) * (SPG_NP_C * nf) : (size_t)0);
+    for (int e = tid; e < SPG_NP_C * nf; e += NT) {
+      const int c = e / nf, k = e - c * nf;
+      const double xk = Gs[k * Cg + nf] / M;
+      double a = 0.0;
+#pragma unroll 1
+      for (int jj = 0; jj < nf; ++jj) a = fma((double)p.W1[(long)c * nf + jj], Gs[jj * Cg + k] - Gs[jj * Cg + nf] * xk, a);
+      out[e] = (float)(-(double)cs[3 * SPG_NP_C + c] * a * (p.fold.grad_mul > 0.0 ? p.fold.grad_mul : 1.0));
+    }
+    return;
+  }
+  if constexpr (PER_SP) {
+    const bool want_dT = p.dT != nullptr;
+    if (want_dT) {
+      const int part = tid & 7, nout = 2 * nf + 2;
+      for (int o0 = 0; o0 < nout; o0 += NT / 8) {
+        const int o = o0 + (tid >> 3);
+        double a = 0.0;
+        if (o < nout) {
+          const bool isk2 = o >= 2 * nf;
+          const int n = isk2 ? o - 2 * nf : o / nf, k = isk2 ? 0 : o - n * nf;
+          for (int c = part; c < SPG_NP_C; c += 8) {
+            const double wn = (double)p.W1[(long)c * nf + n];
+            a = isk2 ? fma((double)cs[c] * (double)cs[SPG_NP_C + c], wn, a) : fma((double)p.W1[(long)c * nf + k] * (double)cs[3 * SPG_NP_C + c], wn, a);
+          }
+        }
+        a += spg_shfl_xor_d(a, 4); a += spg_shfl_xor_d(a, 2); a += spg_shfl_xor_d(a, 1);
+        if (o < nout && part == 0) {
+          if (o >= 2 * nf) k2[o - 2 * nf] = (float)a; else vn[o / nf][o - (o / nf) * nf] = (float)a;
+        }
+      }
+    }
+    __syncthreads();
+    const float un0 = cs[lane] * w1n[0], un1 = cs[lane] * w1n[1];
+    const int total = ((int)gridDim.x - 1) * NW, tps = P / 64;
+    f32x4 dw[4];
+#pragma unroll
+    for (int i = 0; i < 4; ++i) dw[i] = f32x4{0.f, 0.f, 0.f, 0.f};
+#pragma unroll 1
+    for (int g = (int)blockIdx.x * NW + wave; g < p.B; g += total) {
+      f32x4 qr[4];
+#pragma unroll
+      for (int i = 0; i < 4; ++i) qr[i] = f32x4{0.f, 0.f, 0.f, 0.f};
+      for (int j = 0; j < tps; ++j) {
+        const f32x4* qt = reinterpret_cast<const f32x4*>(p.q + ((long)g * tps + j) * (SPG_NP_C * 16) + lane * 16);
+#pragma unroll
+        for (int i = 0; i < 4; ++i) qr[i] += __builtin_nontemporal_load(qt + i);
+      }
+#pragma unroll
+      for (int i = 0; i < 4; ++i) dw[i] += qr[i];
+      if (want_dT) {
+        f32x4 T = f32x4{0.f, 0.f, 0.f, 0.f};
+        if (p.stnT != nullptr) T = *reinterpret_cast<const f32x4*>(p.stnT + (long)g * 4);
+        float s00 = 0.f, s01 = 0.f, s10 = 0.f, s11 = 0.f;
+        const float* xc = p.clouds + (long)g * p.Ctot * P;
+        for (int row = lane; row < P; row += 64) {
+          const float x0 = xc[row], x1 = xc[P + row];
+          float tx = x0, ty = x1;
+          if (p.stnT != nullptr) { tx = fmaf(x0, T[0] + 1.f, x1 * T[2]); ty = fmaf(x0, T[1], x1 * (T[3] + 1.f)); }
+          float e0 = k2[0], e1 = k2[1];
+          e0 = fmaf(tx - xbar[0], vn[0][0], e0); e1 = fmaf(tx - xbar[0], vn[1][0], e1);
+          e0 = fmaf(ty - xbar[1], vn[0][1], e0); e1 = fmaf(ty - xbar[1], vn[1][1], e1);
+          for (int k = 2; k < nf; ++k) {
+            const float xk = xc[(long)k * P + row] - xbar[k];
+            e0 = fmaf(xk, vn[0][k], e0); e1 = fmaf(xk, vn[1][k], e1);
+          }
+          s00 = fmaf(x0, e0, s00); s01 = fmaf(x0, e1, s01); s10 = fmaf(x1, e0, s10); s11 = fmaf(x1, e1, s11);
+        }
+        const float a00 = spg_wave_sum(un0 * qr[3][2] - s00), a01 = spg_wave_sum(un1 * qr[3][2] - s01);
+        const float a10 = spg_wave_sum(un0 * qr[3][3] - s10), a11 = spg_wave_sum(un1 * qr[3][3] - s11);
+        if (lane == 0) { float* o = p.dT + (long)g * 4; o[0] = a00; o[1] = a01; o[2] = a10; o[3] = a11; }
+      }
+    }
+#pragma unroll
+    for (int i = 0; i < 4; ++i)
+#pragma unroll
+      for (int e = 0; e < 4; ++e) red[(wave * SPG_NP_C + lane) * 16 + 4 * i + e] = dw[i][e];
+    __syncthreads();
+    float* out = p.partial + (size_t)blockIdx.x * (SPG_NP_C * nf);
+    for (int e = tid; e < SPG_NP_C * 16; e += NT) {
+      const int c = e >> 4, k = e & 15;
+      if (k < nf) {
+        float a = red[e];
+#pragma unroll
+        for (int w = 1; w < NW; ++w) a += red[w * SPG_NP_C * 16 + e];
+        out[c * nf + k] = cs[c] * a;
+      }
+    }
+  }
+}
+
 }
 
 bool spg_narrow_pair_supported(int nfeat, int c1, int c2, int P, long M) {
@@ -644,3 +770,19 @@
   SPG_LAUNCH_CHECK();
   return 0;
 }
+
+static std::atomic<long> g_fused_launches{0};
+extern "C" long spg_first_conv_fused_launches(int reset) {
+  return reset ? g_fused_launches.exchange(0) : g_fused_launches.load();
+}
+
+int spg_launch_first_conv_finish(const SpgFirstConvFinishParams& p, hipStream_t stream) {
+  ++g_fused_launches;
+  SPG_CHECK_ARG(p.clouds && p.W1 && p.gram && p.partial && p.fold.slots && p.fold.consts && p.fold.C == SPG_NP_C, "first-convolution finish arguments");
+  SPG_CHECK_ARG(p.nfeat >= 2 && p.nfeat + 2 <= 16 && p.P % 64 == 0 && (p.q != nullptr || p.dT == nullptr), "first-convolution finish shape");
+  SpgProfSpan prof(stream, 2.0 * (double)p.B * p.P * SPG_NP_C * (p.nfeat + (p.dT != nullptr ? 2 : 0)), 5000000 + 2, SPG_NP_C, p.nfeat);
+  if (p.q != nullptr) hipLaunchKernelGGL((spg_first_conv_finish_kernel<true>), dim3(fcb_grid(p.B) + 1), dim3(64 * SPG_FCB_NW), 0, stream, p);
+  else hipLaunchKernelGGL((spg_first_conv_finish_kernel<false>), dim3(1), dim3(64 * SPG_FCB_NW), 0, stream, p);
+  SPG_LAUNCH_CHECK();
+  return 0;
+}
diff --git a/superpoint_graph_amd/csrc/spg_pointnet.hip b/superpoint_graph_amd/csrc/spg_pointnet.hip
--- a/superpoint_graph_amd/csrc/spg_pointnet.hip
+++ b/superpoint_graph_amd/csrc/spg_pointnet.hip
@@ -355,7 +355,10 @@
     wmax = (size_t)l.cin * l.cout > wmax ? (size_t)l.cin * l.cout : wmax;
     workmax += ((spg_wgrad_workspace_floats(l.conv ? pl.M : pl.B, l.cout, l.cin) + 63) & ~(size_t)63) + 64 * (size_t)l.cout + 128 +
                ((spg_wgrad_colsum_floats(l.conv ? pl.M : pl.B, l.cout, l.cin) + 63) & ~(size_t)63);
-    if (l.conv && l.cin <= SPG_GRAM_MAXF) workmax += ((size_t)spg_first_conv_bwd_partials(pl.B) * l.cout * l.cin + 63) & ~(size_t)63;
+    if (l.conv && l.cin <= SPG_GRAM_MAXF) {
+      const int fused = pl.M >= 64 ? spg_bwdpair_grid(pl.M, 64) + 1 : 0, parts = spg_first_conv_bwd_partials(pl.B);
+      workmax += ((size_t)(fused > parts ? fused : parts) * l.cout * l.cin + 63) & ~(size_t)63;
+    }
   }
   s.dzA = cv.take<float>((size_t)pl.M * cconv); s.dzB = cv.take<float>((size_t)pl.M * cconv);
   s.fzA = cv.take<float>((size_t)pl.B * cfc); s.fzB = cv.take<float>((size_t)pl.B * cfc);
@@ -447,6 +450,8 @@
   }
   float* dz[2] = {s.dzA, s.dzB};
   flip = 0;
+  bool fused_first = false;
+  SpgPairFirstConv fused_fc; memset(&fused_fc, 0, sizeof(fused_fc));
   for (int k = (int)sg.convs.size() - 1; k >= 0; --k) {
     Layer& l = pl.L[sg.convs[k]];
     if (k > 0 && pl.fold) {
@@ -460,13 +465,40 @@
       g.mmean = prod.mean; g.mrstd = prod.rstd; g.stat_slots = prod.slots_bwd; g.fold_bwd = pending;
       const SpgOperand xin = input_operand(pl, sg, false, k, clouds, stnT);
       if (spg_bwdpair_supported(g, xin)) {
-        SPG_TRY(spg_queue_bwdpair(rq, g, xin, l.dW, st));
+        SpgPairFirstConv fc; memset(&fc, 0, sizeof(fc));
+        Layer& l0 = pl.L[sg.convs[0]];
+        if (k == 1 && sg.convs.size() > 2 && sg.gram != nullptr && gram_recorded(sg.gram) && (!want_dxy || dT_out != nullptr) &&
+            !spg_tune_get(SPG_TUNE_NO_FIRST_CONV_FUSED) && spg_narrow_pair_supported(l0.cin, l0.cout, l.cout, pl.P, pl.M) &&
+            spg_first_conv_bwd_supported(l0.cin, l0.cout, pl.P, pl.M)) {
+          fc.clouds = clouds; fc.stnT = stnT; fc.gram = sg.gram; fc.P = pl.P; fc.Ctot = pl.cfg.nfeat; fc.nfeat = l0.cin;
+          fc.rows = (double)pl.M; fc.per_tile = want_dxy ? 1 : 0;
+          if (want_dxy) fc.q = out; else fc.dW1 = l0.dW;
+          fused_first = spg_bwdpair_first_conv_supported(g, fc);
+        }
+        SPG_TRY(spg_queue_bwdpair(rq, g, xin, l.dW, st, fused_first ? &fc : nullptr));
+        fused_fc = fc;
         if (l.db) SPG_TRY(zero_async(l.db, l.cout, st));
         flip ^= 1;
         pending = fold_bwd_of(pl, prod, pl.M, s.consts);
         cur = op_bnbwd(out, prod.y, prod.ldy, s.consts, prod.cout);
         continue;
       }
+    }
+    if (k == 0 && fused_first) {
+      SPG_CHECK_ARG(pending.slots != nullptr && cur.c0 == s.consts, "first-layer contraction without the pair's pending sums");
+      SpgFirstConvFinishParams fp; memset(&fp, 0, sizeof(fp));
+      fp.clouds = clouds; fp.stnT = stnT; fp.B = pl.B; fp.P = pl.P; fp.Ctot = pl.cfg.nfeat; fp.nfeat = l.cin;
+      fp.W1 = l.W; fp.gram = sg.gram; fp.fold = pending; memset(&pending, 0, sizeof(pending));
+      if (fused_fc.per_tile) {
+        fp.q = fused_fc.q; fp.dT = dT_out;
+        SPG_TRY(spg_queue_partials(rq, spg_first_conv_bwd_partials(pl.B), l.cout * l.cin, l.dW, &fp.partial, st));
+      } else {
+        fp.partial = fused_fc.q + (size_t)(fused_fc.nparts - 1) * l.cout * l.cin;
+      }
+      SPG_TRY(spg_launch_first_conv_finish(fp, st));
+      if (l.db) SPG_TRY(zero_async(l.db, l.cout, st));
+      if (want_dxy && dT_done != nullptr) *dT_done = true;
+      continue;
     }
     if (k == 0 && pl.fold && sg.gram != nullptr && gram_recorded(sg.gram) && sg.convs.size() > 2 && pending.slots != nullptr && cur.mode == SPG_PRO_BNBWD &&
         cur.ld == l.cout && cur.c0 == s.consts && (!want_dxy || dT_out != nullptr) &&
```

Measured after the change: 916,300 superpoints/s. 1.0% lower.
